# Algolzw/image-restoration-sde

Hardware: AMD Instinct MI355X
Metric: restored images/sec at 256x256, 100-step IR-SDE reverse sampler (higher is better)
Workload: dtype f32; 1 GPU; IR-SDE deraining ConditionalUNet nf=64 depth=4, reverse_sde, batch=16/GPU 256x256, T=100 (BASELINE.json configs[1]); compute_dtype=fp32, global_batch=16

## Files before the change

### image_restoration_sde_amd/_lib.py

```python
import ctypes
import os
import subprocess
import threading

_HERE = os.path.dirname(os.path.abspath(__file__))
LIB_PATH = os.environ.get("IRSDE_LIB_PATH") or os.path.join(_HERE, "libirsde_hip.so")
CSRC = os.path.join(_HERE, "csrc")

MODE = {"sde": 0, "ode": 1, "posterior": 2, "dsde_sde": 3, "dsde_ode": 4}
COEF_STRIDE = 12
FLAG_KEEP_ACTIVATIONS = 1
FLAG_NAIVE_CONV = 2
FLAG_NO_WINOGRAD = 4
FLAG_NO_WINOGRAD_F43 = 8
FLAG_UNCOND_FULLATTN = 16
FLAG_BF16 = 32
FLAG_NAF_INTRO_SKIP = 64
FLAG_BF16_ACT = 128
FLAG_NO_FUSED_LN = 256
FLAG_NAF_LENS = 512
FLAG_FP16 = 1024
FLAG_NO_WINOGRAD_FUSED = 2048
FLAG_NO_FUSED_ATTN = 4096
FLAG_NO_NAF_CHAIN = 8192
FLAG_SPLIT_BF16X2 = 16384
FLAG_SPLIT_F16X2 = 32768
FLAG_NAF_STEREO = 65536
FLAG_NAF_UNCOND = 131072
FLAG_UNET_STEREO = 262144
FLAG_F16_ACT = 524288
FLAG_NO_WINO_POLY = 1048576
FLAG_SCAM_STREAM = 2097152
FLAG_NO_SPLIT3 = 4194304
SAMPLE_GRAPH = 1
SAMPLE_PROFILE = 2

SYMBOLS = [
    "irsde_last_error", "irsde_version", "irsde_create", "irsde_create_nafnet", "irsde_destroy", "irsde_num_weights",
    "irsde_weight_name", "irsde_weight_shape", "irsde_load_weight", "irsde_finalize_weights",
    "irsde_set_schedule", "irsde_unet_forward", "irsde_sample", "irsde_sde_step", "irsde_philox_normal",
    "irsde_get_profile", "irsde_debug_tap", "irsde_work_model", "irsde_debug_conv", "irsde_debug_conv_choice", "irsde_debug_conv_halo_choice", "irsde_debug_conv_features", "irsde_plan_describe", "irsde_bench_conv", "irsde_op_profile", "irsde_debug_split_gemm", "irsde_bench_naf_chain", "irsde_debug_force_subbatches", "irsde_debug_force_chain_groups", "irsde_debug_force_wino_poly", "irsde_debug_force_split3", "irsde_debug_force_split3_attn", "irsde_debug_force_split3_blocks", "irsde_debug_scam", "irsde_debug_scam_full",
    "irsde_debug_scam_stream", "irsde_debug_scam_full_stream", "irsde_debug_force_scam_stream",
    "irsde_debug_naf_gate_sca", "irsde_debug_tlsc", "irsde_debug_ln_film", "irsde_debug_naf_lnconv", "irsde_debug_naf_chain", "irsde_debug_naf_chain_split_order",
    "irsde_debug_full_attention16",
    "irsde_eval_metrics", "irsde_tensor2img", "irsde_upscale_bicubic", "irsde_mask_to", "irsde_imresize",
    "irsde_set_lens_info", "irsde_nafnet_set_local_pool", "irsde_create_latent_unet", "irsde_latent_shapes", "irsde_latent_encode", "irsde_latent_decode", "irsde_latent_hidden",
]


class IrsdeLibraryError(RuntimeError):
    pass


class IrsdeError(RuntimeError):
    pass


class Config(ctypes.Structure):
    _fields_ = [("in_nc", ctypes.c_int32), ("out_nc", ctypes.c_int32), ("nf", ctypes.c_int32),
                ("depth", ctypes.c_int32), ("device", ctypes.c_int32), ("flags", ctypes.c_int32)]


class NafConfig(ctypes.Structure):
    _fields_ = [("img_channel", ctypes.c_int32), ("width", ctypes.c_int32), ("middle_blk_num", ctypes.c_int32),
                ("n_enc", ctypes.c_int32), ("enc_blk_nums", ctypes.c_int32 * 8), ("n_dec", ctypes.c_int32),
                ("dec_blk_nums", ctypes.c_int32 * 8), ("device", ctypes.c_int32), ("flags", ctypes.c_int32)]


class LatentConfig(ctypes.Structure):
    _fields_ = [("in_ch", ctypes.c_int32), ("out_ch", ctypes.c_int32), ("ch", ctypes.c_int32), ("n_mult", ctypes.c_int32),
                ("ch_mult", ctypes.c_int32 * 8), ("embed_dim", ctypes.c_int32), ("device", ctypes.c_int32),
                ("flags", ctypes.c_int32)]


_lib = None
_lock = threading.Lock()


PROBES_LIB_PATH = os.path.join(_HERE, "libirsde_hip_probes.so")


def build_library(force=False, verbose=False, probes=True):
    if force:
        subprocess.run(["make", "-C", CSRC, "clean"], check=True, capture_output=not verbose)
    for extra in ([], ["PROBES=1"]) if probes else ([],):
        r = subprocess.run(["make", "-j8", "-C", CSRC] + extra, capture_output=True, text=True)
        if r.returncode != 0:
            raise IrsdeLibraryError("building libirsde_hip%s.so failed:\n" % ("_probes" if extra else "") + r.stdout + r.stderr)
        if verbose:
            print(r.stdout)
    return LIB_PATH


def _declare(lib):
    c = ctypes
    P = c.c_void_p
    lib.irsde_last_error.restype = c.c_char_p
    lib.irsde_last_error.argtypes = []
    lib.irsde_version.restype = c.c_int
    lib.irsde_create.argtypes = [c.POINTER(Config), c.POINTER(P)]
    lib.irsde_create_nafnet.argtypes = [c.POINTER(NafConfig), c.POINTER(P)]
    lib.irsde_destroy.argtypes = [P]
    lib.irsde_destroy.restype = None
    lib.irsde_num_weights.argtypes = [P]
    lib.irsde_weight_name.argtypes = [P, c.c_int]
    lib.irsde_weight_name.restype = c.c_char_p
    lib.irsde_weight_shape.argtypes = [P, c.c_int, c.POINTER(c.c_int64), c.POINTER(c.c_int)]
    lib.irsde_load_weight.argtypes = [P, c.c_char_p, P, c.POINTER(c.c_int64), c.c_int]
    lib.irsde_finalize_weights.argtypes = [P]
    lib.irsde_set_schedule.argtypes = [P, c.c_int, P]
    lib.irsde_unet_forward.argtypes = [P, P, P, c.POINTER(c.c_int64), c.c_int, c.c_int, c.c_int, c.c_int, P, P]
    lib.irsde_sample.argtypes = [P, c.c_int, P, P, P, c.c_uint64, c.c_uint64, c.c_int, c.c_int, c.c_int,
                                 c.c_int, c.c_int, P, P, c.c_int]
    lib.irsde_sde_step.argtypes = [c.c_int, c.c_int, P, P, P, P, P, c.c_uint64, c.c_uint64, c.c_int, c.c_int,
                                   c.c_int, c.c_int, P]
    lib.irsde_philox_normal.argtypes = [P, c.c_int, c.c_int, c.c_int, c.c_uint64, c.c_uint64, P]
    lib.irsde_get_profile.argtypes = [P, c.POINTER(c.c_double)]
    lib.irsde_debug_tap.argtypes = [P, c.c_char_p, P, c.POINTER(c.c_int64)]
    lib.irsde_work_model.argtypes = [P, c.c_int, c.c_int, c.c_int, c.POINTER(c.c_double)]
    lib.irsde_debug_conv.argtypes = [P, c.c_int, P, c.c_int, c.c_int, c.c_int, c.c_int, c.c_int, P, c.c_int, c.c_int,
                                     c.c_int, c.c_int, c.c_int, P, P, c.c_int, c.c_int, P, P, c.c_int, c.c_int, P]
    lib.irsde_debug_conv_choice.argtypes = [c.c_int] * 13 + [c.c_uint] + [c.c_int] * 4 + [c.POINTER(c.c_int), c.c_char_p, c.c_int]
    lib.irsde_debug_conv_halo_choice.argtypes = [c.c_int] * 13 + [c.c_uint] + [c.c_int] * 5 + [c.c_char_p, c.c_int]
    lib.irsde_debug_conv_features.argtypes = ([P, c.c_int, P, c.c_int] + [c.c_int] * 4 + [P] + [c.c_int] * 7 + [P] * 3 + [P, c.c_int, P, P, P, c.c_int] + [c.c_int] * 6 +
                                              [c.POINTER(c.c_int), P, c.c_char_p, c.c_int, P])
    lib.irsde_plan_describe.argtypes = [P, c.c_int, c.c_int, c.c_int, c.c_char_p, c.c_int]
    lib.irsde_op_profile.argtypes = [P, c.c_char_p, c.c_int]
    lib.irsde_bench_conv.argtypes = [c.c_int] * 11 + [c.POINTER(c.c_double)]
    lib.irsde_bench_naf_chain.argtypes = [c.c_int] * 4 + [c.POINTER(c.c_double)]
    lib.irsde_debug_force_subbatches.argtypes = [c.c_int]
    lib.irsde_debug_force_chain_groups.argtypes = [c.c_int]
    lib.irsde_debug_force_wino_poly.argtypes = [c.c_int]
    lib.irsde_debug_force_split3.argtypes = [c.c_int]
    lib.irsde_debug_force_split3_attn.argtypes = [c.c_int]
    lib.irsde_debug_force_split3_blocks.argtypes = [c.c_int]
    lib.irsde_debug_scam.argtypes = [P, c.c_int, c.c_int, c.c_int, c.c_int] + [P] * 12 + [P, P]
    lib.irsde_debug_scam_full.argtypes = [P, c.c_int, c.c_int, c.c_int, c.c_int] + [P] * 12 + [P, P]
    lib.irsde_debug_scam_stream.argtypes = [P, c.c_int, c.c_int, c.c_int, c.c_int] + [P] * 12 + [c.c_int, P, P]
    lib.irsde_debug_scam_full_stream.argtypes = [P, c.c_int, c.c_int, c.c_int, c.c_int] + [P] * 12 + [c.c_int, P, P]
    lib.irsde_debug_force_scam_stream.argtypes = [c.c_int]
    lib.irsde_debug_naf_gate_sca.argtypes = [P, c.c_int, c.c_int, c.c_int, c.c_int] + [P] * 8
    lib.irsde_debug_tlsc.argtypes = [P] + [c.c_int] * 6 + [P] * 4
    lib.irsde_debug_ln_film.argtypes = [P, c.c_int64, c.c_int, c.c_int64, P, P, P, c.c_int, P, P]
    lib.irsde_debug_naf_lnconv.argtypes = [c.c_int, P, c.c_int64, c.c_int, c.c_int, c.c_int64, P, P, P, c.c_int, P, P, P, c.c_int, P, P, P, P, P]
    lib.irsde_debug_naf_chain.argtypes = [P, P, c.c_int, c.c_int] + [P] * 16 + [P, c.c_int, c.c_int, P, c.c_int, c.c_int, c.c_int, P]
    lib.irsde_debug_naf_chain_split_order.argtypes = [c.c_int, c.c_int, c.POINTER(c.c_int), c.c_int64]
    lib.irsde_debug_full_attention16.argtypes = [P, c.c_int, c.c_int, P, P]
    lib.irsde_debug_split_gemm.argtypes = [P, P, P, c.c_int, c.c_int, c.c_int, c.c_int, c.c_int, P]
    lib.irsde_eval_metrics.argtypes = [P, P, c.c_int, c.c_int, c.c_int, c.c_int, c.c_int, c.POINTER(c.c_double), P]
    lib.irsde_tensor2img.argtypes = [P, P, c.c_int, c.c_int, c.c_int, c.c_int, P]
    lib.irsde_upscale_bicubic.argtypes = [P, P, c.c_int, c.c_int, c.c_int, c.c_int, c.c_int, P]
    lib.irsde_mask_to.argtypes = [P, P, c.c_int, c.c_int, c.c_int, c.c_int, P, c.c_int, c.c_int, c.c_int, c.c_int, P]
    lib.irsde_imresize.argtypes = [P, P] + [c.c_int] * 6 + [P, P, c.c_int, P, P, c.c_int, P]
    lib.irsde_set_lens_info.argtypes =[P, c.POINTER(c.c_float), c.c_int]
    lib.irsde_nafnet_set_local_pool.argtypes = [P, c.c_int, c.c_int, c.c_int, c.c_int]
    lib.irsde_create_latent_unet.argtypes = [c.POINTER(LatentConfig), c.POINTER(P)]
    lib.irsde_latent_shapes.argtypes = [P, c.c_int, c.c_int, c.POINTER(c.c_int64), c.POINTER(c.c_int64), c.POINTER(c.c_int)]
    lib.irsde_latent_encode.argtypes = [P, P, c.c_int, c.c_int, c.c_int, P, c.POINTER(P), P]
    lib.irsde_latent_decode.argtypes = [P, P, c.POINTER(P), c.c_int, c.c_int, c.c_int, P, P]
    lib.irsde_latent_hidden.argtypes = [P, c.c_int, c.c_int, c.c_int, c.c_int, P, P]
    for name in SYMBOLS:
        getattr(lib, name)
    return lib


def lib():
    global _lib
    with _lock:
        if _lib is None:
            if not os.path.exists(LIB_PATH):
                raise IrsdeLibraryError(
                    "libirsde_hip.so not found at %s — build it with `python -c 'import __graft_entry__ as g; "
                    "g.build()'` or `make -C %s`. There is no CPU/PyTorch fallback for this path." % (LIB_PATH, CSRC))
            try:
                _lib = _declare(ctypes.CDLL(LIB_PATH))
            except OSError as ex:
                raise IrsdeLibraryError("failed to load %s: %s" % (LIB_PATH, ex)) from ex
        return _lib


_probes = None


def probes_lib():
    global _probes
    with _lock:
        if _probes is None:
            if not os.path.exists(PROBES_LIB_PATH):
                raise IrsdeLibraryError("libirsde_hip_probes.so not found at %s — build it with `make -C %s PROBES=1`" % (PROBES_LIB_PATH, CSRC))
            try:
                _probes = _declare(ctypes.CDLL(PROBES_LIB_PATH))
            except OSError as ex:
                raise IrsdeLibraryError("failed to load %s: %s" % (PROBES_LIB_PATH, ex)) from ex
        return _probes


def check(rc, L=None):
    if rc != 0:
        msg = (L or lib()).irsde_last_error()
        raise IrsdeError("libirsde_hip error %d: %s" % (rc, msg.decode() if msg else "?"))


def stream_ptr(torch_stream=None):
    import torch
    s = torch_stream if torch_stream is not None else torch.cuda.current_stream()
    return ctypes.c_void_p(s.cuda_stream)
```

### image_restoration_sde_amd/csrc/common.h

```cpp
#pragma once
#include <hip/hip_runtime.h>
#include <cstdint>
#include <cstdio>
#include <cstdlib>
#include <stdexcept>
#include <string>
#include <vector>
#include "split3_layout.h"

namespace irsde {

struct HipError : std::runtime_error {
    using std::runtime_error::runtime_error;
};
struct HipOutOfMemory : HipError {
    using HipError::HipError;
};

inline int tuning_env_int(const char* name, int dflt) {
    static const bool on = [] { const char* t = getenv("IRSDE_TUNING"); return t && atoi(t) == 1; }();
    if (!on) return dflt;
    const char* v = getenv(name);
    return v ? atoi(v) : dflt;
}
// ... 35 lines not shown
    const float* zeros = nullptr;
    const float* ch_scale = nullptr;
    const float* in_scale = nullptr;
    int gate = 0;
    const float* gate_film = nullptr;
    int gate_film_bstride = 0;
    int shuffle = 0;
    int nz = 1;
    long long z_in = 0, z_w = 0, z_out = 0;
    int no_direct_epi = 0;
    int in_bf16 = 0, out_bf16 = 0;
    int in_f16 = 0, out_f16 = 0;
    const float* ln_g = nullptr;
    float ln_eps = 1e-5f;
};

struct WinoParams {
    const float* in0 = nullptr;
    const float* in1 = nullptr;
    int C0 = 0, C1 = 0, Hin = 0, Win = 0, in_shift = 0;
    int B = 0, TH = 0, TW = 0, T = 0;
    int tile = 2;
    float* V = nullptr;
    unsigned short* Vs = nullptr;
    int nplanes = 0;
    int v_f16 = 0;
    float v_scale = 1.f;
    int v_pairs = 0;
    int v_triples = 0;
    const float* M = nullptr;
    int Cout = 0;
    float* out = nullptr;
    int out_stride = 0;
    const float* bias = nullptr;
    const float* film = nullptr;
    int film_bstride = 0;
    int silu = 0;
    const float* res = nullptr;
    int res_stride = 0;
};
void launch_wino_input(const WinoParams& p, hipStream_t s);
struct WinoPolyParams {
    int up = 0;
    const float* in = nullptr;
    int C = 0, Hin = 0, Win = 0;
    int B = 0, TH = 0, TW = 0, T = 0;
    float* V = nullptr;
    unsigned short* Vs = nullptr;
    int thread_writer = 0;
    const float* M = nullptr;
    int Cout = 0, Ho = 0, Wo = 0;
    float* out = nullptr;
    int out_stride = 0;
    const float* bias = nullptr;
};
void launch_wino_poly_input(const WinoPolyParams& p, hipStream_t s);
void launch_wino_poly_output(const WinoPolyParams& p, hipStream_t s);
void wino_poly_transform_weights(const float* w_packed, int Cout, int Cin, float* U, int up);
struct SplitGemmArgs {
    const unsigned short* a = nullptr;
    const unsigned short* b = nullptr;
    float* out = nullptr;
    long long plA = 0, plB = 0, pA = 0, pB = 0, pO = 0;
    int M = 0, N = 0, K = 0, lda = 0, ldc = 0;
    float out_scale = 1.f;
    int n_inner = 1;
    int nblk_n = 0;
};
void gemm_split_global_init();
void launch_gemm_split_pairs(const SplitGemmArgs& a, int ncomp, hipStream_t s, int abl = 0, bool f16 = false);
void launch_split_pairs(const float* in, unsigned short* out, size_t rows, int K, hipStream_t s, bool f16 = false,
                        float scale = 1.0f);
struct Split3Launch {
    enum Abl { FULL = 0, NO_LOADS = 1, NO_MFMA = 3, NO_STORES = 4 };
    enum Tri { RULE, ON, OFF };
    Abl abl = FULL;
    Tri walk = RULE;
    Tri drain = RULE;
};
void launch_gemm_split_triples(const SplitGemmArgs& a, int ncomp, hipStream_t s, const Split3Launch& o = {});
void set_force_split3_blocks(int n);
bool gemm_split_triples_fits(long long M, long long N, long long K, long long ldc);
void launch_split_triples(const float* in, unsigned short* out, int ncomp, size_t rows, int K, hipStream_t s);
void launch_split_planes(const float* in, unsigned short* out, size_t n, size_t plane, int nplanes, hipStream_t s, bool f16 = false,
                         float scale = 1.0f);
void launch_wino_output(const WinoParams& p, hipStream_t s);
void wino_transform_weights(const float* w_packed, int Cout, int Cin, float* U, int tile);
bool wino_fused_eligible(const ConvParams& p);
void wino_fused_pack_weights(const float* U, int Cout, int Cin, float* Uf);
void launch_wino_fused(const ConvParams& p, const float* Uf, hipStream_t s, unsigned long long* dbg = nullptr, int dflags = 0);
int wino_fused_num_blocks(const ConvParams& p);
bool wino_fused64_eligible(const ConvParams& p);
void wino_fused64_pack_weights(const float* U, int Cout, int Cin, float* Uf);
void launch_wino_fused64(const ConvParams& p, const float* Uf, hipStream_t s, int variant = 0);
void wino_fused64_set_debug(unsigned long long* buf);
constexpr float kWinoFused64PairVScale = 0.0625f;
void launch_wino_fused64_split_weights(const float* Uf, unsigned short* out, size_t nfloats, float scale, hipStream_t s);
int wino_fused64_num_blocks(const ConvParams& p);
bool wino_fused64_xcd_nb(const ConvParams& p);
void wino_fused_global_init();
int device_cu_count();
bool wino_fused64t_eligible(const ConvParams& p);
long long wino_fused64t_num_items(const ConvParams& p);
void launch_wino_fused64t(const ConvParams& p, const float* Uf, hipStream_t s, int variant = 0);
void wino_fused64t_set_debug(unsigned long long* buf);
void wino_fused_t_global_init();
void naf_chain_global_init();
void naf_chain_set_debug(unsigned long long* buf);
bool naf_chain_shape_ok(int H, int W, int c);
size_t naf_chain_weight_halves(int nblocks);
size_t naf_chain_vec_floats(int nblocks);
void launch_naf_chain(const float* x, float* out, const unsigned short* w, const float* vecs, int nblocks, int B, const float* film, int film_bstride,
                      int film_off, const float* cam, int cam_bstride, int cam_off, hipStream_t s, int variant = 0);
std::vector<int> naf_chain_split_order(int nblocks, int G);
void naf_chain_build_split_weights(const unsigned short* w1, unsigned short* dst, int nblocks, int G, hipStream_t s);
size_t naf_chain_split_scratch_bytes(int B);
int naf_chain_split_groups(int B, int G);
void launch_naf_chain_split(const float* x, float* out, const unsigned short* wG, const float* vecs, int nblocks, int B, const float* film, int film_bstride,
                            int film_off, const float* cam, int cam_bstride, int cam_off, int G, void* scratch, hipStream_t s);
const unsigned* naf_chain_split_error_flag(const void* scratch, int B);
void naf_chain_split_reset(void* scratch, int B);
void naf_chain_set_sabotage(int on);
void attention_global_init();

double conv_flops(const ConvParams& p);
struct ConvTune {
    enum Tile { TILE_AUTO, TILE_128, TILE_256x128, TILE_256, TILE_128_ONE_PER_CU };
    enum Halo { HALO_AUTO, HALO_OFF, HALO_FORCE_512, HALO_FORCE_256 };
    enum ZLoop { ZLOOP_AUTO, ZLOOP_OFF, ZLOOP_ALL, ZLOOP_PAIRS, ZLOOP_FORCE_1X1 };
    enum Order { ORDER_AUTO, ORDER_N_FAST, ORDER_N_SLOW };
    bool rules_off = false;
    Tile tile = TILE_AUTO;
    bool no_buffer_desc = false;
    bool no_direct_epi = false;
    Halo halo = HALO_AUTO;
    ZLoop zloop = ZLOOP_AUTO;
    Order halo_order = ORDER_AUTO;
};
struct ConvKnobs {
    int small_bn = 2, small_bn_f32 = 0;
    int pair_tile256 = 1, pair_inscale256 = 0;
    int no_bufa = 0;
    int zloop = -1, zloop_1x1 = -1;
    int zloop_maxnk = 32, zloop_minblk = 1024, zloop_deep = 1, zloop_ragged64 = 2048;
};
const ConvKnobs& conv_knobs_from_env();
struct HaloChoice {
    int pixels = 0;
    int BN = 0;
    int op = 0, act = 0;
    int tiles_x = 0, tiles_y = 0, nblk_n = 0;
    int n_slow = 0;
    unsigned grid = 0;
    int lds = 0;
    int instance = -1;
};
constexpr int kHaloInstances = 9;
struct ConvChoice {
    enum Family { PAIR, NARROW3, ZLOOP_BATCH, ZLOOP_1X1, HALO, IGEMM };
    enum Operand { OP_F32, OP_F32_BUF, OP_BF16, OP_F16 };
    enum Storage { ACT_F32, ACT_BF16, ACT_F16 };
    Family family = IGEMM;
    int BM = 0, BN = 0;
    Operand op = OP_F32;
    Storage act = ACT_F32;
    bool inscale = false;
// ... 167 lines not shown
```

### image_restoration_sde_amd/csrc/engine.h

```cpp
#pragma once
#include <algorithm>
#include <cmath>
#include <cstring>
#include <functional>
#include <map>
#include <memory>
#include <mutex>
#include <string>
#include <vector>

#include "../../include/irsde_hip.h"
#include "common.h"

namespace irsde {

constexpr int kWinoFusedMaxCin = 256, kWinoFusedMaxCout = 256;
inline long long wino_fused_min_tiles() { return tuning_env_int("IRSDE_WINO_FUSED_MINT", 4096); }
inline bool wino_fused64_enabled() { return tuning_env_int("IRSDE_WINO_FUSED64", 1) != 0; }
inline bool wino_fused64_pair_enabled() { return tuning_env_int("IRSDE_WINO_FUSED64_PAIR", 1) != 0; }
inline int wino_fused64_max_cin() { return tuning_env_int("IRSDE_WINO_FUSED64_MAXCIN", 512); }
inline int wino_fused64_max_cout() { return tuning_env_int("IRSDE_WINO_FUSED64_MAXCOUT", 512); }
inline long long wino_fused64_min_tiles() { return tuning_env_int("IRSDE_WINO_FUSED64_MINT", 1024); }
inline int wino_fused64t_mode() { return tuning_env_int("IRSDE_WINO_FUSED64T", 1); }
inline bool naf_lnconv_enabled() { return tuning_env_int("IRSDE_NAF_LNCONV", 1) != 0; }
inline int naf_chain_split_mode() { return tuning_env_int("IRSDE_NAF_CHAIN_SPLIT", 0); }

int wino_poly_mode();
void set_force_wino_poly(int mode);
constexpr int kWinoPolyUpMinCin = 512;
inline bool wino_poly_wants_weights(int mode, bool up, int Cin) { return mode >= 2 || (mode == 1 && (!up || Cin >= kWinoPolyUpMinCin)); }

int split3_mode();
void set_force_split3(int mode);
constexpr int kSplit3WinoMinCin = 512;
inline int split3_wino_min_cin() { return tuning_env_int("IRSDE_SPLIT3_MINCIN", kSplit3WinoMinCin); }
inline bool split3_wino_wants_weights(int mode, int Cin, int Cout) { return mode >= 2 || Cin > 512 || (Cin >= split3_wino_min_cin() && Cout >= 512); }
inline long long split3_fused_min_tiles() { return tuning_env_int("IRSDE_SPLIT3_FUSED_MINT", 4096); }
constexpr int kSplit3NotExactF32 = IRSDE_FLAG_NO_WINOGRAD | IRSDE_FLAG_NAIVE_CONV | IRSDE_FLAG_BF16 | IRSDE_FLAG_BF16_ACT | IRSDE_FLAG_FP16 | IRSDE_FLAG_F16_ACT |
                                   IRSDE_FLAG_SPLIT_BF16X2 | IRSDE_FLAG_SPLIT_F16X2 | IRSDE_FLAG_NO_SPLIT3;
inline bool split3_wants_weights(int flags) { return !(flags & kSplit3NotExactF32) && split3_mode() > 0; }
int split3_attn_mode();
void set_force_split3_attn(int mode);

inline int wino_min_c(int tile) {
    return tuning_env_int(tile == 4 ? "IRSDE_WINO4_MINC" : "IRSDE_WINO2_MINC", tile == 4 ? 64 : 256);
}

struct DeviceScope {
    int prev = -1;
    explicit DeviceScope(int dev) {
        if (hipGetDevice(&prev) != hipSuccess) prev = -1;
        if (prev != dev) IRSDE_HIP_CHECK(hipSetDevice(dev));
        else prev = -1;
    }
    ~DeviceScope() {
        if (prev >= 0) (void)hipSetDevice(prev);
    }
    DeviceScope(const DeviceScope&) = delete;
    DeviceScope& operator=(const DeviceScope&) = delete;
};

struct HostTensor {
    std::vector<int64_t> shape;
    std::vector<float> data;
    bool loaded = false;
};

struct ConvW {
    float* w = nullptr;
    float* bias = nullptr;
    int Cout = 0, Cin = 0, KH = 1, KW = 1;
    float* wino_u2 = nullptr;
    float* wino_u4 = nullptr;
    float* wino_uf = nullptr;
    float* wino_uf64 = nullptr;
    unsigned short* wino_uf64p = nullptr;
    float wino_uf64p_scale = 1.f;
    unsigned short* wino_up = nullptr;
    float wino_up_scale = 1.f;
    unsigned short* wino_u4t = nullptr;
    unsigned short* wino_polyt = nullptr;
    float* wino_poly = nullptr;
};
struct ResW {
    ConvW b1, b2, res;
    bool has_res = false;
    float* mlp_w = nullptr;
    float* mlp_b = nullptr;
    int film_off = 0;
    int Cout = 0;
};
struct ScamW {
    int c = 0;
    float *gl = nullptr, *gr = nullptr;
    ConvW l, r;
    float *beta = nullptr, *gamma = nullptr;
};
struct AttnW {
    float* g1 = nullptr;
    ConvW qkv, out;
    float* g2 = nullptr;
    int C = 0;
};

struct NafBlockW {
    int c = 0;
    float *g1 = nullptr, *g2 = nullptr;
    ConvW conv1, conv3, conv4, conv5;
    float *dw_w = nullptr, *dw_b = nullptr;
    float *sca_w = nullptr, *sca_b = nullptr;
    float *beta = nullptr, *gamma = nullptr;
    float *mlp_w = nullptr, *mlp_b = nullptr;
    int film_off = 0;
    float *cam_w = nullptr, *cam_b = nullptr;
    int cam_off = 0;
    ScamW fusion;
};

struct NafChainW {
    unsigned short* w = nullptr;
    float* vecs = nullptr;
    int nblocks = 0, film_off = 0, cam_off = 0;
    unsigned short* wsplit[5] = {nullptr, nullptr, nullptr, nullptr, nullptr};
};

// ... 226 lines not shown
    ScamW mid_scam;
    std::vector<ResW> up_res;
    std::vector<AttnW> up_attn;
    std::vector<ConvW> up_conv;
    ResW final_res;
    std::vector<ResW*> all_res;
    int film_row = 0;

    int arch = 0;
    int naf_ic = 0;
    std::vector<int> naf_enc_nums, naf_dec_nums;
    int naf_mid_num = 0;
    std::vector<std::vector<NafBlockW>> naf_enc, naf_dec;
    std::vector<NafBlockW> naf_mid;
    std::vector<ConvW> naf_downs, naf_ups;
    ConvW naf_intro, naf_ending;
    std::vector<NafBlockW*> naf_all;
    std::vector<NafChainW> naf_chain_enc, naf_chain_dec;
    NafChainW naf_chain_mid;
    float *cm_w1 = nullptr, *cm_b1 = nullptr, *cm_w3 = nullptr, *cm_b3 = nullptr;
    int cam_row = 0;
    float* cam_cur = nullptr;
    int cam_rows = 0;
    int cam_set = 0;

    int tlsc_base_h = 0, tlsc_base_w = 0, tlsc_train_h = 0, tlsc_train_w = 0;

    int lat_in = 0, lat_out = 0, lat_ch = 0, lat_embed = 0;
    std::vector<int> lat_mult;
    ConvW lat_init, lat_latent, lat_post, lat_final;
    std::vector<ResW> lat_enc_res, lat_dec_res;
    AttnW lat_enc_attn, lat_dec_attn;
    std::vector<ConvW> lat_down, lat_up;
    std::vector<std::unique_ptr<LatentPlan>> lat_plans;

    int T = 0;
    float* coef_table = nullptr;
    float* film_table = nullptr;
    float* film_cur = nullptr;
    int film_cur_rows = 0;
    StepState* step = nullptr;
    SampleCtl* ctl = nullptr;

    float* zeros = nullptr;
    hipStream_t stream = nullptr;
    hipEvent_t ev_in = nullptr, ev_out = nullptr;
    static constexpr int kMaxSub = 4;
    hipStream_t sub_stream[kMaxSub - 1] = {nullptr, nullptr, nullptr};
    hipEvent_t ev_fork = nullptr, ev_join[kMaxSub - 1] = {nullptr, nullptr, nullptr};
    std::vector<std::unique_ptr<Plan>> plans;
    uint64_t use_counter = 0;
    double profile[12] = {0};
    std::vector<double> op_ms;
    std::vector<std::string> op_desc;
    int op_steps = 0;
    int plan_parts = 1;
    int op_split = 1;
    std::vector<hipEvent_t> ev_pool;
    std::mutex mu;

    float* dmalloc(size_t n) {
        float* p = nullptr;
        IRSDE_HIP_CHECK(hipMalloc(&p, std::max<size_t>(n, 16) * sizeof(float)));
        dev_allocs.push_back(p);
        return p;
    }
    std::map<const float*, unsigned short*> bf16_copies;
    const unsigned short* bf16_copy(const float* w, size_t n) {
        auto it = bf16_copies.find(w);
        if (it != bf16_copies.end()) return it->second;
        unsigned short* d = nullptr;
        IRSDE_HIP_CHECK(hipMalloc(&d, n * sizeof(unsigned short)));
        if (cfg.flags & IRSDE_FLAG_FP16) launch_f32_to_f16(w, d, n, stream);
        else launch_f32_to_bf16(w, d, n, stream);
        IRSDE_HIP_CHECK(hipStreamSynchronize(stream));
        bf16_copies[w] = d;
        return d;
    }
    struct PairCopy { unsigned short* p; float inv_scale; };
    std::map<const float*, PairCopy> pair_copies;
    PairCopy pair_copy(const float* w, size_t n) {
        return make_pair_copy(pair_copies, w, n, [&](unsigned short* d, bool f16, float sc) { launch_split_planes(w, d, n, n, 2, stream, f16, sc); });
    }
    std::map<const float*, unsigned short*> triple_copies;
    const unsigned short* triple_copy(const float* w, size_t rows, int K) {
        const size_t n = rows * (size_t)K;
        auto it = triple_copies.find(w);
        if (it != triple_copies.end()) return it->second;
        unsigned short* d = nullptr;
        IRSDE_HIP_CHECK(hipMalloc(&d, 3 * n * sizeof(unsigned short)));
        dev_allocs.push_back(reinterpret_cast<float*>(d));
        launch_split_frag3(w, d, rows, K, stream);
        IRSDE_HIP_CHECK(hipStreamSynchronize(stream));
        triple_copies[w] = d;
        return d;
    }
    std::map<const float*, PairCopy> pair_copies_il;
    PairCopy pair_copy_il(const float* w, size_t rows, int K) {
        return make_pair_copy(pair_copies_il, w, rows * (size_t)K, [&](unsigned short* d, bool f16, float sc) { launch_split_pairs(w, d, rows, K, stream, f16, sc); });
    }
    template <class Split>
    PairCopy make_pair_copy(std::map<const float*, PairCopy>& cache, const float* w, size_t n, Split split) {
        auto it = cache.find(w);
        if (it != cache.end()) return it->second;
        const bool f16 = (cfg.flags & IRSDE_FLAG_SPLIT_F16X2) != 0;
        float sc = 1.f;
        if (f16) {
            std::vector<float> h(n);
            IRSDE_HIP_CHECK(hipMemcpy(h.data(), w, n * sizeof(float), hipMemcpyDeviceToHost));
            sc = pow2_scale_into_512(h.data(), n);
        }
        unsigned short* d = nullptr;
        IRSDE_HIP_CHECK(hipMalloc(&d, 2 * n * sizeof(unsigned short)));
        dev_allocs.push_back(reinterpret_cast<float*>(d));
        split(d, f16, sc);
        IRSDE_HIP_CHECK(hipStreamSynchronize(stream));
        const PairCopy pc{d, 1.0f / sc};
        cache[w] = pc;
        return pc;
    }
    float* upload(const std::vector<float>& v) {
        float* p = dmalloc(v.size());
        IRSDE_HIP_CHECK(hipMemcpy(p, v.data(), v.size() * sizeof(float), hipMemcpyHostToDevice));
        return p;
    }
};

namespace irsde {

inline bool naf_lens(const irsde_engine* e) { return (e->cfg.flags & IRSDE_FLAG_NAF_LENS) != 0; }
inline bool naf_stereo(const irsde_engine* e) { return e->arch == 1 && (e->cfg.flags & IRSDE_FLAG_NAF_STEREO) != 0; }
inline bool unet_stereo(const irsde_engine* e) { return e->arch == 0 && (e->cfg.flags & IRSDE_FLAG_UNET_STEREO) != 0; }
inline bool stereo_engine(const irsde_engine* e) { return naf_stereo(e) || unet_stereo(e); }
inline bool uncond_engine(const irsde_engine* e) {
    return (e->arch == 0 && (e->cfg.flags & IRSDE_FLAG_UNCOND_FULLATTN) != 0) || (e->arch == 1 && (e->cfg.flags & IRSDE_FLAG_NAF_UNCOND) != 0);
}
inline int rup32(int c) { return (c + 31) & ~31; }
inline bool tlsc_window(const irsde_engine* e, int level, int* K0, int* K1) {
    if (e->tlsc_train_h <= 0) return false;
    const int P = 1 << e->cfg.depth;
    const int Hp = (e->tlsc_train_h + P - 1) / P * P, Wp = (e->tlsc_train_w + P - 1) / P * P;
    *K0 = (int)((long long)(Hp >> level) * e->tlsc_base_h / e->tlsc_train_h);
    *K1 = (int)((long long)(Wp >> level) * e->tlsc_base_w / e->tlsc_train_w);
    return true;
}
inline StepState* step_of(const irsde_engine* e, const Plan* pl) { return pl->own_step ? pl->own_step : e->step; }
inline float* film_of(const irsde_engine* e, const Plan* pl) { return pl->own_film ? pl->own_film : e->film_cur; }

void build_inventory(irsde_engine* e);
void build_inventory_naf(irsde_engine* e);
void build_inventory_latent(irsde_engine* e);
void finalize(irsde_engine* e);
void compute_film_rows(irsde_engine* e, const float* tvals, int rows, float* dst, hipStream_t s);
void ensure_film_cur(irsde_engine* e, int rows);
void pack_conv_rows(const float* w_oihw, const float* bias, int O, int I, int KH, int KW, const std::vector<int>& perm, std::vector<float>& pw,
                    std::vector<float>& pb);
std::vector<int> naf_gate_perm(int c);
std::vector<int> naf_shuffle_perm(int Cout);
std::vector<float> pack_dwconv_taps(const float* w, int c2);
void pack_naf_chain_host(const std::vector<NafChainHostW>& blocks, std::vector<unsigned short>& w, std::vector<float>& vecs);

Plan* get_plan(irsde_engine* e, int B, int H, int W, bool per_sample_film, int slot = 0, int b0 = 0);
int naf_subbatches(const irsde_engine* e, int B, int H, int W);
void set_force_chain_groups(int g);
void set_force_scam_stream(int block_w);
int forced_chain_groups();
int forced_scam_stream();
void set_force_subbatches(int n);
LatentPlan* get_latent_plan(irsde_engine* e, int B, int H, int W, bool decode);

int guard(const std::function<void()>& f);

}
```

### image_restoration_sde_amd/csrc/engine_debug.hip

```cpp
#include "engine.h"
#include "../../include/irsde_hip_debug.h"

using namespace irsde;

namespace irsde {
namespace {

struct Scratch {
    hipStream_t s;
    std::vector<void*> bufs;
    explicit Scratch(hipStream_t s_) : s(s_) {}
    ~Scratch() {
        (void)hipStreamSynchronize(s);
        for (void* p : bufs) (void)hipFree(p);
    }
    Scratch(const Scratch&) = delete;
    Scratch& operator=(const Scratch&) = delete;
    template <class T> T* alloc(size_t n) {
        void* p = nullptr;
        IRSDE_HIP_CHECK(hipMalloc(&p, n * sizeof(T)));
        bufs.push_back(p);
        return static_cast<T*>(p);
    }
    float* upload(const float* host, size_t n) {
// ... 4 lines not shown
    float* upload(const std::vector<float>& v) { return upload(v.data(), v.size()); }
};
struct OwnedStream {
    hipStream_t s = nullptr;
    explicit OwnedStream(unsigned flags) { IRSDE_HIP_CHECK(hipStreamCreateWithFlags(&s, flags)); }
    ~OwnedStream() { (void)hipStreamDestroy(s); }
    OwnedStream(const OwnedStream&) = delete;
    OwnedStream& operator=(const OwnedStream&) = delete;
};
struct EventPair {
    hipEvent_t e0 = nullptr, e1 = nullptr;
    EventPair() {
        IRSDE_HIP_CHECK(hipEventCreate(&e0));
        IRSDE_HIP_CHECK(hipEventCreate(&e1));
    }
    ~EventPair() {
        if (e0) (void)hipEventDestroy(e0);
        if (e1) (void)hipEventDestroy(e1);
    }
    EventPair(const EventPair&) = delete;
    EventPair& operator=(const EventPair&) = delete;
};
template <class Run>
double time_launches(hipStream_t s, int iters, Run&& run) {
    EventPair ev;
    IRSDE_HIP_CHECK(hipEventRecord(ev.e0, s));
    for (int i = 0; i < iters; ++i) run();
    IRSDE_HIP_CHECK(hipEventRecord(ev.e1, s));
    IRSDE_HIP_CHECK(hipStreamSynchronize(s));
    float ms = 0.f;
    IRSDE_HIP_CHECK(hipEventElapsedTime(&ms, ev.e0, ev.e1));
    return ms / iters;
}


ConvTune conv_tune_from_code(int code) {
    ConvTune t;
    t.rules_off = code != 0;
    switch (code) {
        case 3: t.tile = ConvTune::TILE_256x128; break;
        case 50: t.tile = ConvTune::TILE_256; break;
        case 5: t.tile = ConvTune::TILE_128_ONE_PER_CU; break;
        case 6: t.no_buffer_desc = true; break;
        case 7: t.no_direct_epi = true; break;
        case 60: t.tile = ConvTune::TILE_256; t.halo = ConvTune::HALO_OFF; break;
        case 61: t.tile = ConvTune::TILE_128; t.halo = ConvTune::HALO_OFF; break;
        case 64: t.halo = ConvTune::HALO_FORCE_512; break;
        case 65: t.halo = ConvTune::HALO_FORCE_256; break;
        case 68: t.halo = ConvTune::HALO_FORCE_512; t.halo_order = ConvTune::ORDER_N_SLOW; break;
        case 69: t.halo = ConvTune::HALO_FORCE_256; t.halo_order = ConvTune::ORDER_N_SLOW; break;
        case 70: t.zloop = ConvTune::ZLOOP_OFF; break;
        case 71: t.zloop = ConvTune::ZLOOP_ALL; break;
        case 72: t.zloop = ConvTune::ZLOOP_PAIRS; break;
        case 73: t.zloop = ConvTune::ZLOOP_FORCE_1X1; break;
        default: break;
    }
    return t;
}

Split3Launch split3_launch_twin(int twin, int abl = 0) {
    Split3Launch o;
    o.abl = static_cast<Split3Launch::Abl>(abl);
    o.walk = twin == 0 ? Split3Launch::RULE : twin == 1 ? Split3Launch::OFF : Split3Launch::ON;
    o.drain = twin == 0 ? Split3Launch::RULE : twin == 1 ? Split3Launch::OFF : Split3Launch::ON;
    return o;
}

enum class Operand { F32, BF16, F16 };

enum class ConvPath {
    Direct,
    Valu,
    WinoF2,
    WinoF4,
    Poly,
    PolyTriples,
    F4Triples,
    F4Pairs,
    DirectPair,
    Fused32,
    Fused64,
    Fused64Pair,
    Fused64T,
};
struct DebugConvRow {
    int code;
    ConvPath path;
    Operand op;
    bool act_bf16;
    int tune;
    int variant;
    bool up;
    bool thread_writer;
};
constexpr DebugConvRow direct(int code, Operand op, bool act_bf16, int tune) { return {code, ConvPath::Direct, op, act_bf16, tune, 0, false, false}; }
constexpr DebugConvRow on_path(int code, ConvPath path, Operand op = Operand::F32) { return {code, path, op, false, 0, 0, false, false}; }
constexpr DebugConvRow wino(int code, ConvPath path, int tune) { return {code, path, Operand::F32, false, tune, 0, false, false}; }
constexpr DebugConvRow poly(int code, ConvPath path, bool up, bool thread_writer = false) { return {code, path, Operand::F32, false, 0, 0, up, thread_writer}; }
constexpr DebugConvRow fused(int code, ConvPath path, int variant) { return {code, path, Operand::F32, false, 0, variant, false, false}; }
constexpr DebugConvRow kDebugConv[] = {
    direct(0, Operand::F32, false, 0),
    on_path(1, ConvPath::Valu),
    wino(2, ConvPath::WinoF2, 0), wino(12, ConvPath::WinoF2, 71), wino(22, ConvPath::WinoF2, 72),
    wino(3, ConvPath::WinoF4, 0), wino(13, ConvPath::WinoF4, 71), wino(23, ConvPath::WinoF4, 72),
    poly(24, ConvPath::Poly, false), poly(25, ConvPath::Poly, true),
    poly(26, ConvPath::PolyTriples, false), poly(27, ConvPath::PolyTriples, true), poly(28, ConvPath::PolyTriples, true, true),
    on_path(48, ConvPath::F4Triples),
    on_path(44, ConvPath::F4Pairs, Operand::F16), on_path(45, ConvPath::F4Pairs, Operand::BF16),
    on_path(46, ConvPath::DirectPair, Operand::F16), on_path(47, ConvPath::DirectPair, Operand::BF16),
    on_path(33, ConvPath::Fused32),
    fused(34, ConvPath::Fused64, 0), fused(36, ConvPath::Fused64, 64), fused(55, ConvPath::Fused64, 20),
    fused(35, ConvPath::Fused64Pair, 4), fused(37, ConvPath::Fused64Pair, 4 + 64), fused(56, ConvPath::Fused64Pair, 24),
    fused(62, ConvPath::Fused64T, 0), fused(63, ConvPath::Fused64T, 64),
    direct(4, Operand::BF16, false, 0), direct(160, Operand::BF16, false, 60), direct(161, Operand::BF16, false, 61), direct(162, Operand::BF16, false, 64),
    direct(163, Operand::BF16, false, 65),
    direct(5, Operand::F16, false, 0), direct(165, Operand::F16, false, 61), direct(166, Operand::F16, false, 64), direct(167, Operand::F16, false, 65),
    direct(204, Operand::BF16, true, 0), direct(260, Operand::BF16, true, 60), direct(261, Operand::BF16, true, 61), direct(262, Operand::BF16, true, 64),
    direct(263, Operand::BF16, true, 65),
    direct(100, Operand::F32, false, 0), direct(103, Operand::F32, false, 3), direct(105, Operand::F32, false, 5), direct(106, Operand::F32, false, 6),
    direct(107, Operand::F32, false, 7), direct(150, Operand::F32, false, 50), direct(170, Operand::F32, false, 70), direct(171, Operand::F32, false, 71),
    direct(172, Operand::F32, false, 72), direct(173, Operand::F32, false, 73),
};

enum class BenchKind {
    Conv,
    Fused32,
    Fused32Stamps,
    Wino3,
    Wino3Gemm,
    Fused64,
    Fused64Stamps,
    Fused64T,
    Fused64TStamps,
    PairGemm,
    TripleGemm,
};
struct BenchRow {
    int lo, hi;
    BenchKind kind;
    int arg;
    Operand op;
    bool pair;
    bool act_bf16;
};
constexpr BenchRow bench(int lo, int hi, BenchKind kind, int arg, Operand op = Operand::F32, bool pair = false, bool act_bf16 = false) {
    return {lo, hi, kind, arg, op, pair, act_bf16};
}
constexpr BenchRow kBenchConv[] = {
    bench(0, 0, BenchKind::Conv, 0), bench(3, 3, BenchKind::Conv, 3), bench(5, 7, BenchKind::Conv, 5), bench(50, 50, BenchKind::Conv, 50),
    bench(70, 73, BenchKind::Conv, 70),
    bench(60, 61, BenchKind::Conv, 60, Operand::BF16),
    bench(62, 62, BenchKind::Conv, 0, Operand::BF16),
    bench(63, 63, BenchKind::Conv, 0, Operand::BF16, false, true),
    bench(64, 65, BenchKind::Conv, 64, Operand::BF16),
    bench(66, 67, BenchKind::Conv, 64, Operand::BF16, false, true),
    bench(480, 480, BenchKind::Conv, 0, Operand::F16, true), bench(481, 481, BenchKind::Conv, 0, Operand::BF16, true),
    bench(482, 482, BenchKind::Conv, 61, Operand::F16, true),
    bench(80, 80, BenchKind::Fused32, 0),
    bench(83, 82 + 255, BenchKind::Fused32, 1),
    bench(82, 82, BenchKind::Fused32Stamps, 0),
    bench(81, 81, BenchKind::Wino3, 0), bench(421, 421, BenchKind::Wino3Gemm, 0),
    bench(430, 432, BenchKind::Fused64, 20),
    bench(434, 434, BenchKind::Fused64, 24, Operand::F16),
    bench(435, 435, BenchKind::Fused64Stamps, 25), bench(2004, 2004, BenchKind::Fused64Stamps, 25),
    bench(2001, 2002, BenchKind::Fused64Stamps, 28),
    bench(460, 462, BenchKind::Fused64T, 0),
    bench(467, 469, BenchKind::Fused64T, 6),
    bench(465, 465, BenchKind::Fused64TStamps, 5),
    bench(4650, 4653, BenchKind::Fused64TStamps, 12),
    bench(472, 476, BenchKind::PairGemm, 0),
    bench(490, 504, BenchKind::TripleGemm, 0),
};

template <class Row, size_t N, class Lo, class Hi>
constexpr bool codes_disjoint(const Row (&rows)[N], Lo lo, Hi hi) {
    for (size_t i = 0; i < N; ++i)
        for (size_t j = 0; j < N; ++j)
            if (i != j && lo(rows[i]) <= hi(rows[j]) && lo(rows[j]) <= hi(rows[i])) return false;
    return true;
}
constexpr int row_code(const DebugConvRow& r) { return r.code; }
constexpr int row_lo(const BenchRow& r) { return r.lo; }
constexpr int row_hi(const BenchRow& r) { return r.hi; }
static_assert(codes_disjoint(kDebugConv, row_code, row_code), "irsde_debug_conv: a selector code has two rows");
static_assert(codes_disjoint(kBenchConv, row_lo, row_hi), "irsde_bench_conv: a variant has two rows");

const DebugConvRow& debug_conv_lookup(int code) {
    for (const DebugConvRow& r : kDebugConv)
        if (r.code == code) return r;
    throw HipError("debug_conv: unknown selector code " + std::to_string(code));
}
struct BenchSel {
    const BenchRow& row;
    int arg;
};
BenchSel bench_conv_lookup(int code) {
    for (const BenchRow& r : kBenchConv)
        if (code >= r.lo && code <= r.hi) return {r, r.arg + (code - r.lo)};
    throw HipError("bench_conv: unknown variant " + std::to_string(code));
}

SplitGemmArgs split_gemm_args(const unsigned short* a, const unsigned short* b, float* C, int M, int N, int K, size_t pA, size_t pB) {
    SplitGemmArgs g;
    g.a = a; g.b = b; g.out = C;
    g.pA = (long long)pA; g.pB = (long long)pB; g.pO = (long long)M * N;
    g.M = M; g.N = N; g.K = K; g.lda = K; g.ldc = N;
    return g;
}
SplitGemmArgs split_triples(Scratch& mem, const float* A, const float* Bm, float* C, int M, int N, int K, int ncomp, hipStream_t s) {
    const size_t ea = split3_comp_elems((size_t)M, (size_t)K), eb = split3_comp_elems((size_t)N, (size_t)K);
    unsigned short *ta = mem.alloc<unsigned short>(ea * ncomp), *tb = mem.alloc<unsigned short>(eb * ncomp);
    launch_split_triples(A, ta, ncomp, (size_t)M, K, s);
    launch_split_triples(Bm, tb, ncomp, (size_t)N, K, s);
    return split_gemm_args(ta, tb, C, M, N, K, ea, eb);
}
SplitGemmArgs split_pairs(Scratch& mem, const float* A, const float* Bm, float* C, int M, int N, int K, int ncomp, hipStream_t s, bool f16 = false, float sa = 1.f,
                          float sb = 1.f) {
    unsigned short *pa = mem.alloc<unsigned short>((size_t)2 * ncomp * M * K), *pb = mem.alloc<unsigned short>((size_t)2 * ncomp * N * K);
    launch_split_pairs(A, pa, (size_t)ncomp * M, K, s, f16, sa);
    launch_split_pairs(Bm, pb, (size_t)ncomp * N, K, s, f16, sb);
    SplitGemmArgs g = split_gemm_args(pa, pb, C, M, N, K, (size_t)M * K, (size_t)N * K);
    g.out_scale = 1.0f / (sa * sb);
    return g;
}

void write_choice_line(const ConvChoice& c, char* out, int out_len) {
    snprintf(out, (size_t)out_len, "name=%s family=%d tile=%dx%d op=%d act=%d inscale=%d zbatch=%d zrows=%d grid=%ux%ux%u threads=%d lds=%d row=%d of %d",
             c.name().c_str(), (int)c.family, c.BM, c.BN, (int)c.op, (int)c.act, (int)c.inscale, c.zbatch, c.zrows, c.gx, c.gy, c.gz, c.threads, c.lds, c.row,
             conv_instance_count());
}

void write_halo_line(const HaloChoice& h, char* out, int out_len) {
    snprintf(out, (size_t)out_len, "kernel=halo%d bn=%d op=%d act=%d tiles=%dx%d nblk_n=%d nslow=%d grid=%u lds=%d instance=%d of %d", h.pixels, h.BN, h.op, h.act,
             h.tiles_x, h.tiles_y, h.nblk_n, h.n_slow, h.grid, h.lds, h.instance, kHaloInstances);
}

ConvParams choice_hook_params(int B, int Hin, int Win, int C0, int C1, int Cout, int K, int stride, int pad, int in_shift, int operand, int storage, int pair,
                              unsigned features, int splits, int nz) {
    static const float dummy[4] = {};
    float* const some = const_cast<float*>(dummy);
    auto bit = [&](int i) { return (features >> i & 1u) ? some : nullptr; };
    ConvParams p;
    p.in0 = some; p.C0 = C0; p.pix0 = C0; p.in1 = C1 ? some : nullptr; p.C1 = C1; p.pix1 = C1;
    p.Hin = Hin; p.Win = Win; p.in_shift = in_shift;
    p.w = some; p.Cout = Cout; p.KH = K; p.KW = K; p.stride = stride; p.pad_y = pad; p.pad_x = pad;
    p.B = B;
    p.Ho = ((Hin << in_shift) + 2 * pad - K) / stride + 1;
    p.Wo = ((Win << in_shift) + 2 * pad - K) / stride + 1;
    p.out = some; p.out_stride = Cout; p.res_stride = Cout; p.zeros = some;
    p.bias = bit(0); p.film = bit(1); p.silu = bit(2) != nullptr; p.res = bit(3); p.in_scale = bit(4); p.ch_scale = bit(5);
    p.gate = bit(6) != nullptr; p.shuffle = bit(7) != nullptr; p.ln_g = bit(8);
    if (pair) p.w_pair = reinterpret_cast<const unsigned short*>(some);
    else if (operand) p.w_bf = reinterpret_cast<const unsigned short*>(some);
    p.f16 = operand == 2;
// ... 306 lines not shown
        const int Cin = C0 + C1;
        std::vector<float> pk((size_t)Cout * KH * KW * Cin);
        for (int o = 0; o < Cout; ++o)
            for (int i = 0; i < Cin; ++i)
                for (int ky = 0; ky < KH; ++ky)
                    for (int kx = 0; kx < KW; ++kx)
                        pk[(((size_t)o * KH + ky) * KW + kx) * Cin + i] = w_oihw[(((size_t)o * Cin + i) * KH + ky) * KW + kx];
        Scratch mem(s);
        float* dw = mem.upload(pk);
        float* db = bias ? mem.upload(bias, Cout) : nullptr;
        ConvParams p;
        p.in0 = in0; p.C0 = C0; p.pix0 = C0; p.in1 = in1; p.C1 = C1; p.pix1 = C1;
        p.Hin = Hin; p.Win = Win; p.in_shift = in_shift;
        p.w = dw; p.Cout = Cout; p.KH = KH; p.KW = KW; p.stride = stride; p.pad_y = pad; p.pad_x = pad;
        p.B = B;
        p.Ho = ((Hin << in_shift) + 2 * pad - KH) / stride + 1;
        p.Wo = ((Win << in_shift) + 2 * pad - KW) / stride + 1;
        p.out = out; p.out_stride = Cout; p.bias = db; p.film = film; p.film_bstride = film_bstride; p.silu = silu;
        p.res = res; p.res_stride = Cout;
        float* dz = mem.alloc<float>(256);
        IRSDE_HIP_CHECK(hipMemset(dz, 0, 1024));
        p.zeros = dz;
        if (splits > 1 && r.path != ConvPath::Valu && r.path != ConvPath::WinoF2 && r.path != ConvPath::WinoF4) {
            p.splits = splits;
            p.partial = mem.alloc<float>((size_t)splits * B * p.Ho * p.Wo * Cout);
        }
        auto wino_weights = [&](int tile) {
            std::vector<float> U((size_t)(tile + 2) * (tile + 2) * Cout * Cin);
            wino_transform_weights(pk.data(), Cout, Cin, U.data(), tile);
            return U;
        };
        auto wino_tiles = [&](int tile) { return (long long)B * (p.Ho / tile) * (p.Wo / tile); };
        auto alloc_M = [&](int ncomp, long long T) { return mem.alloc<float>((size_t)ncomp * T * Cout); };
        auto poly_plan = [&](const char* refusal, float*& dU) {
            if (!(r.up ? wino_poly_up_shape(p) : wino_poly_down_shape(p)) || !wino_poly_eligible(p) || splits > 1) throw HipError(refusal);
            std::vector<float> U((size_t)100 * Cout * Cin);
            wino_poly_transform_weights(pk.data(), Cout, Cin, U.data(), r.up);
            dU = mem.upload(U);
            return make_wino_poly(p, dU, nullptr, nullptr);
        };
        switch (r.path) {
        case ConvPath::PolyTriples: {
            float* dU = nullptr;
            WinoPolyPlan wp = poly_plan("debug_conv: selectors 26 / 27 / 28 run what 24 / 25 run (single source, channels a multiple of 32, bias only)", dU);
            if (!gemm_split_triples_fits(wp.T, Cout, wp.K, Cout)) throw HipError("debug_conv: shape not eligible for the three-piece GEMM");
            unsigned short* dUt = mem.alloc<unsigned short>((size_t)wp.ncomp * split3_comp_elems((size_t)Cout, (size_t)wp.K));
            unsigned short* dVt = mem.alloc<unsigned short>((size_t)wp.ncomp * split3_comp_elems((size_t)wp.T, (size_t)wp.K));
            float* dM = alloc_M(wp.ncomp, wp.T);
            launch_split_triples(dU, dUt, wp.ncomp, (size_t)Cout, wp.K, s);
            wp = make_wino_poly(p, dU, nullptr, dM);
            const SplitGemmArgs sg = make_wino_poly_triples(wp, Cout, dUt, dVt, dM);
            wp.in.thread_writer = r.thread_writer;
            launch_wino_poly_input(wp.in, s);
            launch_gemm_split_triples(sg, wp.ncomp, s);
            launch_wino_poly_output(wp.out, s);
            break;
        }
        case ConvPath::Poly: {
            float* dU = nullptr;
            WinoPolyPlan wp = poly_plan(r.up ? "debug_conv: selector 25 runs a 3x3 stride-1 pad-1 convolution with in_shift = 1 (single source, channels a multiple of 32, bias only)"
                                             : "debug_conv: selector 24 runs a 4x4 stride-2 pad-1 convolution (single source, channels a multiple of 32, bias only)", dU);
            float* dV = mem.alloc<float>((size_t)wp.ncomp * wp.T * wp.K);
            wp = make_wino_poly(p, dU, dV, alloc_M(wp.ncomp, wp.T));
            launch_wino_poly_input(wp.in, s);
            launch_conv(wp.gemm, s);
            launch_wino_poly_output(wp.out, s);
            break;
        }
        case ConvPath::F4Triples: {
            if (!wino_shape_ok(p, 4) || Cin % 32) throw HipError("debug_conv: shape not eligible for the three-piece GEMM");
            const std::vector<float> U = wino_weights(4);
            const long long T = wino_tiles(4);
            if (!gemm_split_triples_fits(T, Cout, Cin, Cout)) throw HipError("debug_conv: shape not eligible for the three-piece GEMM");
            float* dU = mem.upload(U);
            unsigned short* dUt = mem.alloc<unsigned short>((size_t)36 * split3_comp_elems((size_t)Cout, (size_t)Cin));
            unsigned short* dVt = mem.alloc<unsigned short>((size_t)36 * split3_comp_elems((size_t)T, (size_t)Cin));
            launch_split_triples(dU, dUt, 36, (size_t)Cout, Cin, s);
            const WinoSplitPlan sp = make_wino_triples(p, dUt, dVt, alloc_M(36, T));
            launch_wino_input(sp.in, s);
            launch_gemm_split_triples(sp.gemm, 36, s);
            launch_wino_output(sp.out, s);
            break;
        }
        case ConvPath::F4Pairs: {
            const bool f16 = r.op == Operand::F16;
            if (!wino_shape_ok(p, 4) || Cin % 32) throw HipError("debug_conv: shape not eligible for the pair GEMM");
            std::vector<float> U = wino_weights(4);
            const float us = f16 ? pow2_scale_into_512(U.data(), U.size()) : 1.f;
            const long long T = wino_tiles(4);
            float* dU = mem.upload(U);
            unsigned short* dUp = mem.alloc<unsigned short>(2 * U.size());
            unsigned short* dVp = mem.alloc<unsigned short>((size_t)36 * T * Cin * 2);
            launch_split_pairs(dU, dUp, (size_t)36 * Cout, Cin, s, f16, us);
            const WinoSplitPlan sp = make_wino_pairs(p, dUp, dVp, alloc_M(36, T), f16, us);
            launch_wino_input(sp.in, s);
            launch_gemm_split_pairs(sp.gemm, 36, s, 0, f16);
            launch_wino_output(sp.out, s);
            break;
        }
        case ConvPath::Fused64Pair: {
            if (!wino_fused64_eligible(p)) throw HipError("debug_conv: shape not eligible for the fused Winograd kernel");
            std::vector<float> U = wino_weights(4), Uf(U.size());
            wino_fused64_pack_weights(U.data(), Cout, Cin, Uf.data());
            const float usc = pow2_scale_into_512(U.data(), U.size());
            float* dUf = mem.upload(Uf);
            unsigned short* dUp = mem.alloc<unsigned short>(2 * Uf.size());
            launch_wino_fused64_split_weights(dUf, dUp, Uf.size(), usc, s);
            p.pair_scale = 1.0f / (kWinoFused64PairVScale * usc);
            launch_wino_fused64(p, reinterpret_cast<const float*>(dUp), s, r.variant);
            break;
        }
        case ConvPath::Fused32:
        case ConvPath::Fused64:
        case ConvPath::Fused64T: {
            const bool f32k = r.path == ConvPath::Fused32;
            if (f32k ? !wino_fused_eligible(p) : !wino_fused64_eligible(p)) throw HipError("debug_conv: shape not eligible for the fused Winograd kernel");
            const std::vector<float> U = wino_weights(4);
            std::vector<float> Uf(U.size());
            if (f32k) wino_fused_pack_weights(U.data(), Cout, Cin, Uf.data());
            else wino_fused64_pack_weights(U.data(), Cout, Cin, Uf.data());
            float* dUf = mem.upload(Uf);
            if (r.path == ConvPath::Fused64T) {
                if (!wino_fused64t_eligible(p)) throw HipError("debug_conv: shape not eligible for the two-tile-group fused Winograd kernel");
                launch_wino_fused64t(p, dUf, s, r.variant);
            } else if (f32k) {
                launch_wino_fused(p, dUf, s);
            } else {
                launch_wino_fused64(p, dUf, s, r.variant);
            }
            break;
        }
        case ConvPath::WinoF2:
        case ConvPath::WinoF4: {
            const int tile = r.path == ConvPath::WinoF2 ? 2 : 4, ncomp = (tile + 2) * (tile + 2);
            if (!wino_shape_ok(p, tile)) throw HipError("debug_conv: shape not eligible for Winograd");
            const std::vector<float> U = wino_weights(tile);
            const long long T = wino_tiles(tile);
            float* dU = mem.upload(U);
            float* dV = mem.alloc<float>((size_t)ncomp * T * Cin);
            const WinoPlan wp = make_wino(p, dU, dV, alloc_M(ncomp, T), tile);
            launch_wino_input(wp.in, s);
            launch_conv(wp.gemm, s, conv_tune_from_code(r.tune));
            launch_wino_output(wp.out, s);
            break;
        }
        case ConvPath::DirectPair: {
            const bool f16 = r.op == Operand::F16;
            const float sc = f16 ? pow2_scale_into_512(pk.data(), pk.size()) : 1.f;
            unsigned short* dwp = mem.alloc<unsigned short>(2 * pk.size());
            launch_split_pairs(dw, dwp, (size_t)Cout, KH * KW * (C0 + C1), s, f16, sc);
            p.w_pair = dwp; p.pair_scale = 1.0f / sc; p.f16 = f16 ? 1 : 0;
            launch_conv(p, s);
            break;
        }
        case ConvPath::Valu:
            launch_conv_naive(p, s);
            break;
        case ConvPath::Direct: {
            unsigned short* ao = nullptr;
            if (r.op != Operand::F32) {
                unsigned short* d16 = mem.alloc<unsigned short>(pk.size());
                if (r.op == Operand::F16) launch_f32_to_f16(dw, d16, pk.size(), s);
                else launch_f32_to_bf16(dw, d16, pk.size(), s);
                p.w_bf = d16;
                p.f16 = r.op == Operand::F16 ? 1 : 0;
            }
// ... 112 lines not shown
            wsc = f16 ? pow2_scale_into_512(pk.data(), pk.size()) : 1.f;
            w16 = mem.alloc<unsigned short>(2 * pk.size());
            p.w_pair = w16; p.pair_scale = 1.0f / wsc;
        } else if (operand) {
            w16 = mem.alloc<unsigned short>(pk.size());
            p.w_bf = w16;
        }
        p.f16 = f16 ? 1 : 0;
        if (storage) {
            a0 = mem.alloc<unsigned short>(npix_in * C0);
            p.in0 = reinterpret_cast<const float*>(a0);
            if (in1) { a1 = mem.alloc<unsigned short>(npix_in * C1); p.in1 = reinterpret_cast<const float*>(a1); }
            if (res) { ar = mem.alloc<unsigned short>(nout); p.res = reinterpret_cast<const float*>(ar); }
            ao = mem.alloc<unsigned short>(nout);
            p.out = reinterpret_cast<float*>(ao);
            p.in_bf16 = p.out_bf16 = storage == 1;
            p.in_f16 = p.out_f16 = storage == 2;
        }
        ConvKnobs k;
        static_assert(sizeof(ConvKnobs) == 11 * sizeof(int), "the hook's knob array is ConvKnobs, field by field");
        if (knobs) memcpy(&k, knobs, sizeof k);
        conv_validate(p);
        auto narrow = [&](const float* src, unsigned short* dst, size_t n) {
            if (storage == 2) launch_f32_to_f16(src, dst, n, s);
            else launch_f32_to_bf16(src, dst, n, s);
        };
        if (pair) launch_split_pairs(dw, w16, (size_t)Cout * nz, K * K * Cin, s, f16, wsc);
        else if (operand == 2) launch_f32_to_f16(dw, w16, pk.size(), s);
        else if (operand == 1) launch_f32_to_bf16(dw, w16, pk.size(), s);
        if (storage) {
            narrow(in0, a0, npix_in * C0);
            if (in1) narrow(in1, a1, npix_in * C1);
            if (res) narrow(res, ar, nout);
            IRSDE_HIP_CHECK(hipMemsetAsync(ao, 0xFF, nout * 2, s));
        }
        ConvChoice c;
        launch_conv(p, s, conv_tune_from_code(tune), knobs ? &k : nullptr, &c);
        if (storage == 2) launch_f16_to_f32(ao, out, nout, s);
        else if (storage == 1) launch_bf16_to_f32(ao, out, nout, s);
        IRSDE_HIP_CHECK(hipStreamSynchronize(s));
        write_choice_line(c, choice, choice_len);
        if (c.family == ConvChoice::HALO) {
            const size_t n = strlen(choice);
            if (n + 2 < (size_t)choice_len) {
                choice[n] = ' ';
                write_halo_line(c.halo, choice + n + 1, choice_len - (int)n - 1);
            }
        }
    });
}

int irsde_debug_split_gemm(const float* A, const float* Bm, float* C, int M, int N, int K, int ncomp, int nplanes, void* stream) {
    return guard([&] {
        const int twin3 = nplanes == 43 ? 0 : nplanes == 45 ? 1 : nplanes == 47 ? 2 : -1;
        if (twin3 < 0 && nplanes != 42 && nplanes != 44) throw HipError("debug_split_gemm: nplanes must be 42, 43, 44, 45 or 47");
        hipStream_t s = reinterpret_cast<hipStream_t>(stream);
        conv_global_init();
        Scratch mem(s);
        if (twin3 >= 0) {
            if (!gemm_split_triples_fits(M, N, K, N)) throw HipError("debug_split_gemm: shape not eligible for the three-piece GEMM");
            launch_gemm_split_triples(split_triples(mem, A, Bm, C, M, N, K, ncomp, s), ncomp, s, split3_launch_twin(twin3));
        } else {
            const bool f16 = nplanes == 44;
            launch_gemm_split_pairs(split_pairs(mem, A, Bm, C, M, N, K, ncomp, s, f16, f16 ? 1.0f / 16.0f : 1.f, f16 ? 64.0f : 1.f), ncomp, s, 0, f16);
        }
        IRSDE_HIP_CHECK(hipStreamSynchronize(s));
    });
}

int irsde_debug_force_chain_groups(int g) {
    set_force_chain_groups(g == 1 || g == 2 || g == 4 ? g : 0);
    return IRSDE_OK;
}

int irsde_debug_force_split3(int mode) {
    set_force_split3(mode >= 0 && mode <= 2 ? mode : -1);
    return IRSDE_OK;
}

int irsde_debug_force_split3_attn(int mode) {
    set_force_split3_attn(mode >= 0 && mode <= 2 ? mode : -1);
    return IRSDE_OK;
}
int irsde_debug_force_split3_blocks(int n) {
    if (n >= 0 && n < 8) return guard([&] { throw HipError("debug_force_split3_blocks: n must be at least 8 (one block per XCD), or negative for the default"); });
    set_force_split3_blocks(n);
    return IRSDE_OK;
}

int irsde_debug_force_wino_poly(int mode) {
    set_force_wino_poly(mode >= 0 && mode <= 2 ? mode : -1);
    return IRSDE_OK;
}

int irsde_debug_force_subbatches(int n) {
    set_force_subbatches(n < 0 ? 0 : n);
    return IRSDE_OK;
}

int irsde_bench_naf_chain(int variant, int nblocks, int B, int iters, double* ms_out) {
    return guard([&] {
        if (!ms_out || nblocks < 1 || nblocks > 64 || B < 1 || iters < 1) throw HipError("bench_naf_chain: bad argument");
        const int G = variant == 22 ? 2 : (variant == 24 || variant == 25 || variant == 26) ? 4 : 1;
#ifdef IRSDE_PROBES
        if (variant != 0 && variant != 1 && variant != 11 && G == 1) throw HipError("bench_naf_chain: bad variant");
#else
        if (variant != 0 && variant != 1 && G == 1) throw HipError("bench_naf_chain: variant 11 is a measurement twin (make PROBES=1)");
#endif
        conv_global_init();
        OwnedStream stream(hipStreamDefault);
        hipStream_t s = stream.s;
        Scratch mem(s);
        const size_t nx = (size_t)B * 64 * 512, nw = naf_chain_weight_halves(nblocks), nv = naf_chain_vec_floats(nblocks);
        float *dx = mem.alloc<float>(nx), *dout = mem.alloc<float>(nx), *dvec = mem.alloc<float>(nv), *dfilm = mem.alloc<float>((size_t)nblocks * 2048);
        unsigned short* dw = mem.alloc<unsigned short>(nw);
        const size_t chunk = (size_t)64 << 20;
        float* dwf = mem.alloc<float>(chunk);
        launch_fill_random(dx, nx, 1, 1.0f, s);
        launch_fill_random(dvec, nv, 2, 0.1f, s);
        launch_fill_random(dfilm, (size_t)nblocks * 2048, 3, 0.1f, s);
        for (size_t o = 0; o < nw; o += chunk) {
            const size_t n = std::min(chunk, nw - o);
            launch_fill_random(dwf, n, 4 + (unsigned)(o / chunk), 0.04f, s);
            launch_f32_to_f16(dwf, dw + o, n, s);
        }
        unsigned short* dwg = nullptr;
        void* dscratch = nullptr;
        if (G > 1) {
            IRSDE_HIP_CHECK(hipStreamSynchronize(s));
            dwg = mem.alloc<unsigned short>(nw);
            naf_chain_build_split_weights(dw, dwg, nblocks, G, s);
            dscratch = mem.alloc<char>(naf_chain_split_scratch_bytes(B));
            IRSDE_HIP_CHECK(hipMemset(dscratch, 0, naf_chain_split_scratch_bytes(B)));
        }
        auto run = [&]() {
            if (G > 1) launch_naf_chain_split(dx, dout, dwg, dvec, nblocks, B, dfilm, 0, 0, nullptr, 0, 0, G, dscratch, s);
            else launch_naf_chain(dx, dout, dw, dvec, nblocks, B, dfilm, 0, 0, nullptr, 0, 0, s, variant == 11 ? 1 : variant);
        };
        if (variant == 26) {
#ifdef IRSDE_PROBES
            naf_chain_set_sabotage(1);
#else
            throw HipError("bench_naf_chain: variant 26 is a PROBES-build test");
#endif
        }
        struct SabotageOff { ~SabotageOff() { naf_chain_set_sabotage(0); } } sabotage_off;
        run();
        if (variant == 25) {
#ifdef IRSDE_PROBES
            const int ng = naf_chain_split_groups(B, 4);
            unsigned long long* dd = mem.alloc<unsigned long long>((size_t)ng * 8 * 16);
            IRSDE_HIP_CHECK(hipMemsetAsync(dd, 0, (size_t)ng * 8 * 16 * 8, s));
            naf_chain_set_debug(dd);
            run();
            IRSDE_HIP_CHECK(hipStreamSynchronize(s));
            naf_chain_set_debug(nullptr);
            std::vector<unsigned long long> hd((size_t)ng * 8 * 16);
            IRSDE_HIP_CHECK(hipMemcpy(hd.data(), dd, hd.size() * 8, hipMemcpyDeviceToHost));
            double acc[16] = {0};
            double nwv = 0;
            for (size_t w = 0; w < (size_t)ng * 8; ++w) {
                if (!hd[w * 16 + 15]) continue;
                for (int k = 0; k < 16; ++k) acc[k] += (double)hd[w * 16 + k];
                nwv += 1;
            }
            static const char* names[12] = {"norm1 (incl. residual-stream fetch)", "conv1 GEMM passes", "depthwise 3x3 + gate + pool", "gated fetch behind barrier (pool)", "sca.1 GEMM", "conv3 GEMM + residual", "norm2 (incl. residual-stream fetch)", "conv4 GEMM + gate", "conv5 GEMM + residual", "scale-vector / gated fetch (sca, conv4)", "group barriers (6 per block)", "publishing (gated slice, residual slice)"};
            printf("naf_chain stamps, 4 groups per image: %d blocks, B=%d; shader cycles per wave and block (mean over %.0f waves)\n", nblocks, B, nwv);
            for (int k = 0; k < 12; ++k) printf("  %-42s %9.0f\n", names[k], acc[k] / nwv / nblocks);
            printf("  %-42s %9.0f\n", "whole kernel / blocks", acc[15] / nwv / nblocks);
            fflush(stdout);
#else
            throw HipError("bench_naf_chain: variant 25 is a measurement twin (make PROBES=1)");
#endif
        }
        if (variant == 11) {
            unsigned long long* dd = mem.alloc<unsigned long long>((size_t)B * 8 * 16);
            IRSDE_HIP_CHECK(hipMemsetAsync(dd, 0, (size_t)B * 8 * 16 * 8, s));
            naf_chain_set_debug(dd);
            launch_naf_chain(dx, dout, dw, dvec, nblocks, B, dfilm, 0, 0, nullptr, 0, 0, s, 11);
            IRSDE_HIP_CHECK(hipStreamSynchronize(s));
            naf_chain_set_debug(nullptr);
            std::vector<unsigned long long> hd((size_t)B * 8 * 16);
            IRSDE_HIP_CHECK(hipMemcpy(hd.data(), dd, hd.size() * 8, hipMemcpyDeviceToHost));
            double acc[16] = {0};
            for (size_t i = 0; i < hd.size(); ++i) acc[i % 16] += (double)hd[i];
            const double nwv = (double)B * 8, nb = nblocks;
            static const char* names[10] = {"norm1", "conv1 GEMM passes", "depthwise 3x3 + gate + pool", "barrier (pool)", "sca.1 GEMM", "conv3 GEMM + residual", "norm2", "conv4 GEMM + gate", "conv5 GEMM + residual", "barriers (sca, conv4)"};
            printf("naf_chain stamps: %d blocks, B=%d; shader cycles per wave and block (mean over %d waves); MFMA floor per wave: conv1 / conv4 512 x 16, conv3 / conv5 256 x 16, sca 64 x 16\n", nblocks, B, B * 8);
            for (int k = 0; k < 10; ++k) printf("  %-30s %9.0f\n", names[k], acc[k] / nwv / nb);
            printf("  %-30s %9.0f\n", "whole kernel / blocks", acc[15] / nwv / nb);
            fflush(stdout);
        }
        *ms_out = time_launches(s, iters, run);
        if (G > 1) {
            unsigned flag = 0;
            IRSDE_HIP_CHECK(hipMemcpy(&flag, naf_chain_split_error_flag(dscratch, B), 4, hipMemcpyDeviceToHost));
            if (flag) throw HipError("bench_naf_chain: the split kernel's groups were not co-resident (spin timeout)");
        }
    });
}

int irsde_bench_conv(int variant, int B, int H, int W, int Cin, int Cout, int K, int stride, int up, int epi, int iters,
                     double* ms_out) {
    return guard([&] {
        if (!ms_out || iters < 1) throw HipError("bad argument");
        const BenchSel sel = bench_conv_lookup(variant);
        const BenchRow& r = sel.row;
        const BenchKind kind = r.kind;
        const int arg = sel.arg;
        conv_global_init();
        OwnedStream stream(hipStreamNonBlocking);
        hipStream_t s = stream.s;
        Scratch mem(s);
        ConvParams p;
        p.B = B; p.Hin = H; p.Win = W; p.in_shift = up; p.C0 = Cin; p.pix0 = Cin;
        p.Cout = Cout; p.KH = K; p.KW = K; p.stride = stride; p.pad_y = p.pad_x = (K == 4 ? 1 : K / 2);
        p.Ho = ((H << up) + 2 * p.pad_y - K) / stride + 1;
        p.Wo = ((W << up) + 2 * p.pad_x - K) / stride + 1;
        const size_t nin = (size_t)B * H * W * Cin, nw = (size_t)Cout * K * K * Cin, nout = (size_t)B * p.Ho * p.Wo * Cout;
        float *din = mem.alloc<float>(nin), *dw = mem.alloc<float>(nw), *dout = mem.alloc<float>(nout), *dres = mem.alloc<float>(nout);
        float* dfilm = mem.alloc<float>((size_t)2 * Cout + 256);
        float* dz = dfilm + 2 * Cout;
        IRSDE_HIP_CHECK(hipMemset(dz, 0, 1024));
        p.zeros = dz;
        launch_fill_random(din, nin, 1, 1.0f, s);
        launch_fill_random(dw, nw, 2, 1.0f / sqrtf((float)(K * K * Cin)), s);
        launch_fill_random(dres, nout, 3, 1.0f, s);
        launch_fill_random(dfilm, (size_t)2 * Cout, 4, 0.3f, s);
        p.in0 = din; p.w = dw; p.out = dout; p.out_stride = Cout;
        if (kind == BenchKind::Conv && r.op == Operand::BF16 && !r.pair) {
            unsigned short* dbf = mem.alloc<unsigned short>(nw);
            launch_f32_to_bf16(dw, dbf, nw, s);
            p.w_bf = dbf;
        }
        if (epi == 1) { p.film = dfilm; p.silu = 1; }
        if (epi == 2) { p.silu = 1; p.res = dres; p.res_stride = Cout; }
        if (r.act_bf16) {
            unsigned short* dabf = mem.alloc<unsigned short>(nin);
            launch_f32_to_bf16(din, dabf, nin, s);
            launch_f32_to_bf16(dout, reinterpret_cast<unsigned short*>(dres), nout / 2, s);
            p.in0 = reinterpret_cast<const float*>(dabf);
            p.in_bf16 = 1; p.out_bf16 = 1;
        }
        if (r.pair) {
            const bool f16 = r.op == Operand::F16;
            unsigned short* dwp = mem.alloc<unsigned short>(2 * nw);
            launch_split_pairs(dw, dwp, (size_t)Cout, K * K * Cin, s, f16, 64.0f);
            p.w_pair = dwp; p.pair_scale = 1.0f / 64.0f; p.f16 = f16 ? 1 : 0;
        }
        if (kind == BenchKind::TripleGemm || kind == BenchKind::PairGemm) {
            if (K != 3 || stride != 1 || !wino_shape_ok(p, 4)) throw HipError("bench_conv: Winograd variants need an eligible 3x3 stride-1 layer");
            const long long T = (long long)B * (p.Ho / 4) * (p.Wo / 4);
            const bool triples = kind == BenchKind::TripleGemm;
            if (triples && !gemm_split_triples_fits(T, Cout, Cin, Cout)) throw HipError("bench_conv: shape not eligible for the three-piece GEMM");
            float *vf = mem.alloc<float>((size_t)36 * T * Cin), *uf = mem.alloc<float>((size_t)36 * Cout * Cin), *mo = mem.alloc<float>((size_t)36 * T * Cout);
            launch_fill_random(vf, (size_t)36 * T * Cin, 7, 1.0f, s);
            launch_fill_random(uf, (size_t)36 * Cout * Cin, 8, 0.05f, s);
            const SplitGemmArgs g = triples ? split_triples(mem, vf, uf, mo, (int)T, Cout, Cin, 36, s) : split_pairs(mem, vf, uf, mo, (int)T, Cout, Cin, 36, s);
            const Split3Launch twin = split3_launch_twin(arg / 5, arg % 5);
            auto gemms = [&] {
                if (triples) launch_gemm_split_triples(g, 36, s, twin);
                else launch_gemm_split_pairs(g, 36, s, arg);
            };
            for (int i = 0; i < 2; ++i) gemms();
            *ms_out = time_launches(s, iters, gemms);
            return;
        }
        float* dU = nullptr;
        WinoPlan wp{};
        if (kind == BenchKind::Fused32Stamps) {
            dU = mem.alloc<float>((size_t)36 * nw / 9);
            launch_fill_random(dU, (size_t)36 * nw / 9, 5, 1.0f / sqrtf((float)(9 * Cin)), s);
            const int nb = wino_fused_num_blocks(p);
            unsigned long long* dd = mem.alloc<unsigned long long>((size_t)nb * 128);
            launch_wino_fused(p, dU, s);
            IRSDE_HIP_CHECK(hipMemsetAsync(dd, 0, (size_t)nb * 128 * 8, s));
            launch_wino_fused(p, dU, s, dd);
            IRSDE_HIP_CHECK(hipStreamSynchronize(s));
            std::vector<unsigned long long> hd((size_t)nb * 128);
            IRSDE_HIP_CHECK(hipMemcpy(hd.data(), dd, hd.size() * 8, hipMemcpyDeviceToHost));
            double ph[2][4] = {{0, 0, 0, 0}, {0, 0, 0, 0}};
            unsigned long long rt_min = ~0ull, rt_max = 0;
            for (int bi = 0; bi < nb; ++bi)
                for (int w = 0; w < 8; ++w) {
                    const unsigned long long* t = &hd[((size_t)bi * 8 + w) * 16];
                    for (int k = 0; k < 4; ++k) ph[w >= 4][k] += (double)(t[k + 1] - t[k]) / ((double)nb * 4);
                    rt_min = std::min(rt_min, t[7]);
                    rt_max = std::max(rt_max, t[7]);
                }
            printf("wino_fused timeline B=%d %dx%d Cin=%d Cout=%d: %d blocks, block starts span %.1f us\n", B, p.Ho, p.Wo, Cin, Cout, nb,
                   (double)(rt_max - rt_min) / 100.0);
            printf("  MFMA waves     (shader cycles): start->V[0] ready %.0f | K loop %.0f | acc->LDS+barrier %.0f | epilogue %.0f\n", ph[0][0],
                   ph[0][1], ph[0][2], ph[0][3]);
            printf("  producer waves (shader cycles): start->chunk 0 done %.0f | K loop rest %.0f | wait MFMA+acc %.0f | epilogue %.0f\n",
                   ph[1][0], ph[1][1], ph[1][2], ph[1][3]);
            fflush(stdout);
            *ms_out = 0.0;
            return;
        }
        if (kind != BenchKind::Conv) {
            const bool three_launch = kind == BenchKind::Wino3 || kind == BenchKind::Wino3Gemm;
            if (K != 3 || stride != 1) throw HipError("bench_conv: Winograd variants need a 3x3 stride-1 layer");
            dU = mem.alloc<float>((size_t)36 * nw / 9);
            launch_fill_random(dU, (size_t)36 * nw / 9, 5, 1.0f / sqrtf((float)(9 * Cin)), s);
            if (!three_launch && !wino_fused_eligible(p)) throw HipError("bench_conv: shape not eligible for the fused Winograd kernel");
            if (kind != BenchKind::Fused32 && kind != BenchKind::Wino3 && !wino_fused64_eligible(p))
                throw HipError("bench_conv: shape not eligible for the 64-cout fused Winograd kernel");
            if (kind == BenchKind::Fused64 && r.op == Operand::F16) {
                float* dUp = mem.alloc<float>((size_t)36 * nw / 9);
                launch_wino_fused64_split_weights(dU, reinterpret_cast<unsigned short*>(dUp), (size_t)36 * nw / 9, 256.0f, s);
                dU = dUp;
                p.pair_scale = 1.0f / (kWinoFused64PairVScale * 256.0f);
            }
            if (three_launch) {
                if (!wino_shape_ok(p, 4)) throw HipError("bench_conv: shape not eligible for Winograd F(4x4,3x3)");
                const long long T = (long long)B * (p.Ho / 4) * (p.Wo / 4);
                float* dV = mem.alloc<float>((size_t)36 * T * Cin);
                float* dM = mem.alloc<float>((size_t)36 * T * Cout);
                wp = make_wino(p, dU, dV, dM, 4);
                if (kind == BenchKind::Wino3Gemm) launch_wino_input(wp.in, s);
            }
        }
        if (kind == BenchKind::Fused64TStamps) {
            if (!wino_fused64t_eligible(p)) throw HipError("bench_conv: shape not eligible for the two-tile-group fused Winograd kernel");
            const int nbp = 256;
            unsigned long long* dd = mem.alloc<unsigned long long>((size_t)nbp * 64);
            launch_wino_fused64t(p, dU, s, 0);
            IRSDE_HIP_CHECK(hipMemsetAsync(dd, 0, (size_t)nbp * 64 * 8, s));
            wino_fused64t_set_debug(dd);
            launch_wino_fused64t(p, dU, s, arg);
            IRSDE_HIP_CHECK(hipStreamSynchronize(s));
// ... 79 lines not shown
```

### image_restoration_sde_amd/csrc/engine_plan.hip

```cpp
#include "engine.h"
#include <atomic>

using namespace irsde;

namespace irsde {

struct Builder {
    irsde_engine* e;
    Plan* pl;
    bool reuse;
    bool naive;
    int film_bstride;
    int b0 = 0;
    const float* film_base() const { return film_of(e, pl) + (size_t)b0 * film_bstride; }
    const float* cam_base() const { return e->cam_cur + (size_t)b0 * e->cam_row; }
    const float* fused_ln_g = nullptr;

    bool act_bf16() const { return (e->cfg.flags & IRSDE_FLAG_BF16_ACT) != 0; }
    bool act_f16() const { return (e->cfg.flags & IRSDE_FLAG_F16_ACT) != 0; }
    Tensor talloc(int B, int H, int W, int C, int force_f32 = 0) {
        Tensor t;
        t.B = B; t.H = H; t.W = W; t.C = C;
        t.bf16 = act_bf16() && !force_f32;
        t.f16 = act_f16() && !force_f32;
        t.p = pl->alloc(t.half() ? (t.numel() + 1) / 2 : t.numel(), reuse);
        return t;
    }
    void tfree(const Tensor& t) {
        if (reuse) pl->release(t.p);
    }
    void tap(const std::string& name, const Tensor& t) { pl->taps[name] = t; }

    void push_op(Op op) {
        pl->conv_flops += op.flops;
        pl->conv_exec_flops += op.exec_flops;
        pl->conv_bytes += op.bytes;
        pl->net_ops.push_back(std::move(op));
    }

    void push_conv(ConvParams p) {
        const int M = p.B * p.Ho * p.Wo;
        const int bn = conv_base_bn(p.Cout);
        const int blocks = ((M + 127) / 128) * ((p.Cout + bn - 1) / bn);
        const int nk = p.KH * p.KW * ((p.C0 + p.C1) / 32);
        int splits = 1;
        if (!naive && blocks < 256 && nk >= 16 && !p.gate && !p.shuffle) {
            splits = std::min(std::min(nk / 8, (512 + blocks - 1) / blocks), 16);
            if (splits < 2) splits = 1;
        }
        if (splits > 1) {
            p.splits = splits;
            p.partial = pl->alloc((size_t)splits * M * p.Cout, true);
        }
        p.zeros = e->zeros;
        if (!naive && (e->cfg.flags & IRSDE_FLAG_BF16)) {
            p.w_bf = e->bf16_copy(p.w, (size_t)p.Cout * p.KH * p.KW * (p.C0 + p.C1));
            p.f16 = (e->cfg.flags & IRSDE_FLAG_FP16) ? 1 : 0;
        } else if (!naive && (e->cfg.flags & (IRSDE_FLAG_SPLIT_BF16X2 | IRSDE_FLAG_SPLIT_F16X2)) && p.Cout >= 64 && p.nz == 1 && !p.ln_g &&
                   p.KH * p.KW * (p.C0 + p.C1) >= split_direct_min_k()) {
            const auto pc = e->pair_copy_il(p.w, (size_t)p.Cout, p.KH * p.KW * (p.C0 + p.C1));
            p.w_pair = pc.p; p.pair_scale = pc.inv_scale;
            p.f16 = (e->cfg.flags & IRSDE_FLAG_SPLIT_F16X2) ? 1 : 0;
        }
        Op op;
        op.kind = OP_CONV;
        op.flops = conv_flops(p);
        const double in_bytes = (p.in_bf16 || p.in_f16 ? 2.0 : 4.0) * (double)p.B * (p.Hin) * (p.Win) * (double)(p.C0 + p.C1);
        op.bytes = in_bytes + (p.out_bf16 || p.out_f16 ? 2.0 : 4.0) * (double)M * p.Cout +
                   (p.w_bf ? 2.0 : 4.0) * (double)p.Cout * p.KH * p.KW * (p.C0 + p.C1);
        op.exec_flops = op.flops;
        {
            long long launched = blocks;
            std::string kernel;
            if (!naive) {
                const ConvChoice c = conv_choose(p, ConvTune{}, conv_knobs_from_env(), device_cu_count());
                if (c.family == ConvChoice::HALO) kernel = conv_halo2_wanted(p) ? " kernel=halo512" : " kernel=halo256";
                else launched = c.blocks(), kernel = " kernel=" + c.name();
            }
            char buf[256];
            snprintf(buf, sizeof buf, "conv%s M=%d Cout=%d Cin=%d k=%dx%d s=%d up=%d splits=%d blocks=%lld flops=%.4g",
                     p.w_pair ? (p.f16 ? "(split f16x2)" : "(split bf16x2)") : p.w_bf ? (p.f16 ? (p.in_f16 || p.out_f16 ? "(fp16 operands + storage)" : "(fp16)") : "(bf16)") : "", M, p.Cout, p.C0 + p.C1, p.KH, p.KW, p.stride, p.in_shift, splits, launched, op.flops);
            op.desc = buf + kernel;
        }
        const bool nv = naive;
        op.fn = [p, nv](hipStream_t s) {
            if (nv)
                launch_conv_naive(p, s);
            else
                launch_conv(p, s);
        };
        push_op(std::move(op));
        if (p.partial) pl->release(p.partial);
    }

    Tensor conv(const ConvW& w, const Tensor& in0, const Tensor* in1, int stride, int pad, int in_shift,
                const float* film, int silu, const Tensor* res, int out_stride = 0) {
        ConvParams p;
        p.in0 = in0.p; p.C0 = in0.C; p.pix0 = in0.C;
        if (in1) { p.in1 = in1->p; p.C1 = in1->C; p.pix1 = in1->C; }
        if (p.C0 + p.C1 != w.Cin) throw HipError("conv: channel mismatch");
        p.Hin = in0.H; p.Win = in0.W; p.in_shift = in_shift;
        p.w = w.w; p.Cout = w.Cout; p.KH = w.KH; p.KW = w.KW; p.stride = stride; p.pad_y = pad; p.pad_x = pad;
        const int Hv = in0.H << in_shift, Wv = in0.W << in_shift;
        p.B = in0.B;
        p.Ho = (Hv + 2 * pad - w.KH) / stride + 1;
        p.Wo = (Wv + 2 * pad - w.KW) / stride + 1;
        const int ostr = out_stride ? out_stride : w.Cout;
        Tensor out = talloc(p.B, p.Ho, p.Wo, ostr, out_stride != 0);
        p.out = out.p; p.out_stride = ostr;
        p.in_bf16 = in0.bf16; p.out_bf16 = out.bf16;
        p.ln_g = fused_ln_g;
        if ((in1 && in1->bf16 != in0.bf16) || (res && res->bf16 != out.bf16)) throw HipError("conv: mixed activation storage types");
        p.bias = w.bias;
        p.film = film; p.film_bstride = film ? film_bstride : 0;
        p.silu = silu;
        if (res) { p.res = res->p; p.res_stride = res->C; }
        if (!naive) {
            if (w.wino_poly && push_wino_poly(p, w.wino_poly, w.wino_polyt)) return out;
            if (w.wino_up && wino_shape_ok(p, 4) && push_wino(p, w.wino_u4, 4, w.wino_up, w.wino_up_scale)) return out;
            if (split3_over_fused(w, p) && push_wino(p, w.wino_u4, 4, nullptr, 1.f, w.wino_u4t)) return out;
            if (w.wino_uf64p && push_wino_fused(p, reinterpret_cast<const float*>(w.wino_uf64p), true, w.wino_uf64p_scale)) return out;
            if (w.wino_uf64 && push_wino_fused(p, w.wino_uf64, true)) return out;
            if (w.wino_uf && push_wino_fused(p, w.wino_uf, false)) return out;
            if (w.wino_u4 && wino_shape_ok(p, 4) && push_wino(p, w.wino_u4, 4, nullptr, 1.f, w.wino_u4t)) return out;
            if (w.wino_u2 && wino_shape_ok(p, 2) && push_wino(p, w.wino_u2, 2)) return out;
        }
        push_conv(p);
        return out;
    }

    bool push_wino_fused(const ConvParams& d, const float* Uf, bool k64, float pair_uscale = 0.f) {
        ConvParams dd = d;
        dd.zeros = e->zeros;
        if (pair_uscale != 0.f) dd.pair_scale = 1.0f / (kWinoFused64PairVScale * pair_uscale);
        auto eligible = [&](const ConvParams& q) { return k64 ? wino_fused64_eligible(q) : wino_fused_eligible(q); };
        int parts = 1;
        if (!eligible(dd)) {
            for (parts = 2; parts <= 4; parts *= 2) {
                if (d.B % parts) continue;
                ConvParams q = dd;
                q.B = d.B / parts;
                if (eligible(q)) break;
            }
            if (parts > 4) return false;
            dd.B = d.B / parts;
        }
        const int Ctot = d.C0 + d.C1;
        const long long T = (long long)dd.B * (d.Ho / 4) * (d.Wo / 4);
        const long long blocks = k64 ? wino_fused64_num_blocks(dd) : (long long)dd.B * ((d.Ho / 4 + 3) / 4) * ((d.Wo / 4 + 7) / 8) * (d.Cout / 32);
        if (T < (k64 ? wino_fused64_min_tiles() : wino_fused_min_tiles()) || blocks < 256) return false;
        bool use_t = false;
        if (k64 && pair_uscale == 0.f && wino_fused64t_mode() && wino_fused64t_eligible(dd)) {
            const double per_block = (double)wino_fused64t_num_items(dd) / std::max(1, device_cu_count());
            const double work = per_block * (Ctot / 16);
            use_t = wino_fused64t_mode() >= 2 || (!d.in_shift && (work >= 64.0 || (work >= 32.0 && per_block >= 8.0 && !d.res)));
        }
        Op op;
        op.kind = OP_CONV;
        op.flops = conv_flops(d);
        op.exec_flops = 36 * 2.0 * (double)T * parts * Ctot * d.Cout;
        op.bytes = 4.0 * (double)d.B * d.Hin * d.Win * Ctot + 4.0 * (double)d.B * d.Ho * d.Wo * d.Cout + 4.0 * 9.0 * (double)d.Cout * Ctot;
        char buf[256];
        const bool pair = pair_uscale != 0.f;
        snprintf(buf, sizeof buf, "conv(%swinograd F4 fused) %s T=%lld Cout=%d Cin=%d up=%d blocks=%lld flops=%.4g exec=%.4g%s", pair ? "split f16x2 " : "",
                 use_t ? "32x64" : k64 ? "16x64" : "32x32", T * parts, d.Cout, Ctot, d.in_shift, blocks * parts, op.flops, op.exec_flops,
                 parts > 1 ? (parts == 2 ? " (2 batch slices)" : " (4 batch slices)") : "");
        op.desc = buf;
        std::vector<ConvParams> slices;
        for (int i = 0; i < parts; ++i) {
            ConvParams q = dd;
            const size_t b0 = (size_t)i * dd.B;
            q.in0 = dd.in0 + b0 * dd.Hin * dd.Win * dd.pix0;
            if (dd.in1) q.in1 = dd.in1 + b0 * dd.Hin * dd.Win * dd.pix1;
            q.out = dd.out + b0 * dd.Ho * dd.Wo * dd.out_stride;
            if (dd.res) q.res = dd.res + b0 * dd.Ho * dd.Wo * dd.res_stride;
            if (dd.film && dd.film_bstride) q.film = dd.film + b0 * dd.film_bstride;
            slices.push_back(q);
        }
        if (use_t)
            op.fn = [slices, Uf](hipStream_t s) { for (const auto& q : slices) launch_wino_fused64t(q, Uf, s, 0); };
        else if (k64)
            op.fn = [slices, Uf, pair](hipStream_t s) { for (const auto& q : slices) launch_wino_fused64(q, Uf, s, pair ? 4 : 0); };
        else
            op.fn = [slices, Uf](hipStream_t s) { for (const auto& q : slices) launch_wino_fused(q, Uf, s); };
        push_op(std::move(op));
        return true;
    }

    static constexpr long long kSplit3MinRows = 256;
    static constexpr int kSplit3MinCout = 512, kSplit3MinCoutPoly = 256;
    static constexpr double kSplit3MinFlop = 9e9;
    bool split3_rule(long long T, int K, int Cout, int ncomp, int min_cout = kSplit3MinCout) const {
        return T >= kSplit3MinRows && Cout >= min_cout && ncomp * 2.0 * (double)T * K * Cout >= kSplit3MinFlop;
    }
    bool split3_adopts(const unsigned short* Ut, long long T, int K, int Cout, int ncomp, int min_cout = kSplit3MinCout) const {
        const int mode = split3_mode();
        if (!Ut || mode <= 0 || naive || (e->cfg.flags & kSplit3NotExactF32) || !gemm_split_triples_fits(T, Cout, K, Cout)) return false;
        return mode >= 2 || split3_rule(T, K, Cout, ncomp, min_cout);
    }
    bool split3_over_fused(const ConvW& w, const ConvParams& p) const {
        if (!w.wino_u4t || p.C0 + p.C1 > 512 || !wino_shape_ok(p, 4)) return false;
        const long long T = (long long)p.B * (p.Ho / 4) * (p.Wo / 4);
        return T >= split3_fused_min_tiles() && split3_rule(T, p.C0 + p.C1, p.Cout, 36) && split3_adopts(w.wino_u4t, T, p.C0 + p.C1, p.Cout, 36);
    }
    static bool split3_attn_rule(int C, int N, int B) {
        (void)N; (void)B;
        return attn_split3_has_instance(C);
    }
// ... 703 lines not shown
    }
    b.tap("intro", x);
    const bool intro_skip = (e->cfg.flags & IRSDE_FLAG_NAF_INTRO_SKIP) != 0;
    const Tensor intro = x;
    auto run_level = [&](NafChainW& chain, const std::vector<NafBlockW>& blks, const std::string& path, int level) {
        auto advance = [&](const Tensor& y) {
            if (!(intro_skip && x.p == intro.p)) b.tfree(x);
            x = y;
        };
        if (!b.tlsc_local(x, level) && b.naf_chain_ok(chain, x))
            advance(b.nafchain(chain, x));
        else
            for (size_t j = 0; j < blks.size(); ++j) advance(block(blks[j], x, path + std::to_string(j), level));
    };
    std::vector<Tensor> encs;
    for (size_t i = 0; i < e->naf_enc.size(); ++i) {
        run_level(e->naf_chain_enc[i], e->naf_enc[i], "encoders." + std::to_string(i) + ".", (int)i);
        b.tap("encoders." + std::to_string(i), x);
        encs.push_back(x);
        Builder::ConvOpts od;
        od.stride = 2;
        x = b.conv_naf(e->naf_downs[i], x, od);
        b.tap("downs." + std::to_string(i), x);
    }
    const int nlev = (int)e->naf_enc.size();
    run_level(e->naf_chain_mid, e->naf_mid, "middle_blks.", nlev);
    b.tap("middle", x);
    for (size_t i = 0; i < e->naf_dec.size(); ++i) {
        Tensor skip = encs[encs.size() - 1 - i];
        Builder::ConvOpts ou;
        ou.shuffle = 1; ou.res = &skip;
        Tensor y = b.conv_naf(e->naf_ups[i], x, ou);
        b.tfree(x);
        b.tfree(skip);
        x = y;
        b.tap("ups." + std::to_string(i), x);
        run_level(e->naf_chain_dec[i], e->naf_dec[i], "decoders." + std::to_string(i) + ".", nlev - 1 - (int)i);
        b.tap("decoders." + std::to_string(i), x);
    }
    if (intro_skip) {
        Tensor y = b.talloc(x.B, x.H, x.W, x.C);
        const float *xa = x.p, *xb = intro.p;
        float* yo = y.p;
        const size_t n = x.numel();
        b.push_other(OP_OTHER, [=](hipStream_t s) { launch_add(xa, xb, yo, n, s); });
        b.tfree(x);
        b.tfree(intro);
        x = y;
    }
    Builder::ConvOpts oe;
    oe.pad = 1; oe.out_stride = stereo ? (e->naf_ic + 3) & ~3 : pl->pred_stride;
    Tensor pr = b.conv_naf(e->naf_ending, x, oe);
    b.tfree(x);
    if (stereo) {
        float* pred = pl->alloc((size_t)pl->B * pl->Hp * pl->Wp * pl->pred_stride, false);
        const float* src = pr.p;
        const int Bp = pl->B, ic = e->naf_ic, Hp = pl->Hp, Wp = pl->Wp, is = oe.out_stride, os = pl->pred_stride;
        b.push_other(OP_OTHER, [=](hipStream_t s) { launch_stereo_pack_pred(src, pred, Bp, ic, Hp, Wp, is, os, s); });
        pl->net_ops.back().desc = "stereo_pack_pred";
        pl->pred = pred;
        return;
    }
    pl->pred = pr.p;
}

static std::atomic<int> g_force_chain_groups{0};
void set_force_chain_groups(int g) { g_force_chain_groups.store(g, std::memory_order_relaxed); }
int forced_chain_groups() { return g_force_chain_groups.load(std::memory_order_relaxed); }
static std::atomic<int> g_force_scam_stream{0};
void set_force_scam_stream(int block_w) { g_force_scam_stream.store(block_w, std::memory_order_relaxed); }
int forced_scam_stream() { return g_force_scam_stream.load(std::memory_order_relaxed); }
static std::atomic<int> g_force_split3{-1};
void set_force_split3(int mode) { g_force_split3.store(mode, std::memory_order_relaxed); }
int split3_mode() {
    const int f = g_force_split3.load(std::memory_order_relaxed);
    return f >= 0 ? f : tuning_env_int("IRSDE_SPLIT3", 1);
}
static std::atomic<int> g_force_split3_attn{-1};
void set_force_split3_attn(int mode) { g_force_split3_attn.store(mode, std::memory_order_relaxed); }
int split3_attn_mode() {
    const int f = g_force_split3_attn.load(std::memory_order_relaxed);
    return f >= 0 ? f : tuning_env_int("IRSDE_SPLIT3_ATTN", 1);
}
static std::atomic<int> g_force_wino_poly{-1};
void set_force_wino_poly(int mode) { g_force_wino_poly.store(mode, std::memory_order_relaxed); }
int wino_poly_mode() {
    const int f = g_force_wino_poly.load(std::memory_order_relaxed);
    return f >= 0 ? f : tuning_env_int("IRSDE_WINO_POLY", 1);
}
static std::atomic<int> g_force_subbatches{0};
void set_force_subbatches(int n) { g_force_subbatches.store(n, std::memory_order_relaxed); }
int naf_subbatches(const irsde_engine* e, int B, int H, int W) {
    if (e->arch == 2 || stereo_engine(e) || (e->cfg.flags & (IRSDE_FLAG_NAIVE_CONV | IRSDE_FLAG_KEEP_ACTIVATIONS))) return 1;
    int n = g_force_subbatches.load(std::memory_order_relaxed);
    if (n <= 0) {
        static const int env = tuning_env_int("IRSDE_SUBBATCHES", 0);
        n = env;
    }
    if (n <= 0 && e->arch != 1) n = 1;
    if (n <= 0) {
        bool chain = false;
        const int nlev = (int)e->naf_enc.size(), ps = 1 << nlev;
        const int Hp = (H + ps - 1) / ps * ps, Wp = (W + ps - 1) / ps * ps;
        if ((e->cfg.flags & IRSDE_FLAG_FP16) && !(e->cfg.flags & (IRSDE_FLAG_NO_NAF_CHAIN | IRSDE_FLAG_F16_ACT)))
            for (int i = 0; i < nlev; ++i)
                if (e->naf_chain_enc[i].nblocks > 0 && naf_chain_shape_ok(Hp >> i, Wp >> i, e->naf_intro.Cout << i)) {
                    int K0 = 0, K1 = 0;
                    if (!tlsc_window(e, i, &K0, &K1) || (K0 >= (Hp >> i) && K1 >= (Wp >> i))) chain = true;
                }
        n = chain && B >= 8 ? 2 : 1;
    }
    n = std::min(n, (int)irsde_engine::kMaxSub);
    while (n > 1 && B % n) --n;
    return std::max(n, 1);
}

static bool evict_lru_plan(irsde_engine* e) {
    if (e->plans.empty()) return false;
    size_t lru = 0;
    for (size_t i = 1; i < e->plans.size(); ++i)
        if (e->plans[i]->last_use < e->plans[lru]->last_use) lru = i;
    IRSDE_HIP_CHECK(hipDeviceSynchronize());
    const int vb = e->plans[lru]->B, vh = e->plans[lru]->H, vw = e->plans[lru]->W;
    const bool split = e->plans[lru]->slot > 0;
    for (size_t i = e->plans.size(); i-- > 0;)
        if (i == lru || (split && e->plans[i]->slot > 0 && e->plans[i]->B == vb && e->plans[i]->H == vh && e->plans[i]->W == vw))
            e->plans.erase(e->plans.begin() + i);
    return true;
}

static Plan* build_plan(irsde_engine* e, int B, int H, int W, bool per_sample_film, int slot, int b0);

static void init_plan_geometry(irsde_engine* e, Plan* pl, int B, int H, int W, int sdiv) {
    pl->B = B; pl->H = H; pl->W = W;
    pl->Hp = (H + sdiv - 1) / sdiv * sdiv;
    pl->Wp = (W + sdiv - 1) / sdiv * sdiv;
    pl->last_use = ++e->use_counter;
    if (e->arch != 1 && (pl->Hp - H >= H || pl->Wp - W >= W)) throw HipError("image too small for reflect padding");
}

Plan* get_plan(irsde_engine* e, int B, int H, int W, bool per_sample_film, int slot, int b0) {
    for (auto& p : e->plans)
        if (p->B == B && p->H == H && p->W == W && p->per_sample_film == per_sample_film && p->slot == slot && p->b0 == b0) {
            p->last_use = ++e->use_counter;
            return p.get();
        }
    if (e->plans.size() >= 8) evict_lru_plan(e);
    for (;;) {
        try {
            return build_plan(e, B, H, W, per_sample_film, slot, b0);
        } catch (const HipOutOfMemory&) {
            if (!evict_lru_plan(e)) throw;
        }
    }
}

static Plan* build_plan(irsde_engine* e, int B, int H, int W, bool per_sample_film, int slot, int b0) {
    const bool stereo = stereo_engine(e), ustereo = unet_stereo(e);
    if (stereo && slot > 0) throw HipError("internal: a stereo batch is never split into sub-batches");
    ensure_film_cur(e, per_sample_film ? (stereo ? 2 : 1) * (b0 + B) : 1);
    if (naf_lens(e)) {
        if (e->cam_set < b0 + B) throw HipError("latent-bokeh ConditionalNAFNet: irsde_set_lens_info must cover the batch first");
        if (e->cam_rows < b0 + B) throw HipError("internal: lens table smaller than the batch");
    }

    const int depth = e->cfg.depth, nf = e->cfg.nf, in_nc = e->cfg.in_nc;
// ... 236 lines not shown
```

### image_restoration_sde_amd/csrc/gemm_split.hip

```cpp
#include "common.h"
#include <algorithm>
#include <atomic>
#include <type_traits>

namespace irsde {

typedef float floatx16 __attribute__((ext_vector_type(16)));
typedef __bf16 bf16x8 __attribute__((ext_vector_type(8)));
typedef _Float16 f16x8 __attribute__((ext_vector_type(8)));
typedef unsigned uintx4 __attribute__((ext_vector_type(4)));

namespace {

constexpr int SG_BK = 32;

#define IRSDE_GLDS16(GPTR, LPTR) \
    __builtin_amdgcn_global_load_lds((const __attribute__((address_space(1))) void*)(GPTR), (__attribute__((address_space(3))) void*)(LPTR), 16, 0, 0)

template <int ABL = 0, bool F16 = false>
__global__ __launch_bounds__(512, 2) void gemm_split2i_kernel(const SplitGemmArgs g) {
    using frag_t = typename std::conditional<F16, f16x8, bf16x8>::type;
    constexpr int TM = 4, TN = 2, WN = 4, BM = 256, BN = 256;
    constexpr int A_STAGE = BM * 128, STAGE = (BM + BN) * 128;
    extern __shared__ __attribute__((aligned(16))) char lds[];
    const int tid = threadIdx.x, lane = tid & 63;
    const int wave = __builtin_amdgcn_readfirstlane(tid >> 6);
    const int wm = wave / WN, wn = wave % WN;
    const int l31 = lane & 31, h = lane >> 5;
    const int mtiles = (g.M + BM - 1) / BM;
    const int units = mtiles * g.n_inner;
    const int xcd = blockIdx.x & 7, jx = blockIdx.x >> 3;
    const int ulo = (int)((long long)xcd * units / 8), uhi = (int)((long long)(xcd + 1) * units / 8);
    const int unit = ulo + jx / g.nblk_n;
    if (unit >= uhi) return;
    const int nblk = jx % g.nblk_n;
    const int plane0 = unit / mtiles, mblk = unit - plane0 * mtiles;
    const int m0 = mblk * BM, n0 = nblk * BN;
    const int nk = g.K / SG_BK;
    const int steps = nk;
    const unsigned rowb = (unsigned)nk * 128u;

    unsigned a_voff[4], b_voff[4];
#pragma unroll
    for (int ps = 0; ps < 4; ++ps) {
        const int row = (ps * 8 + wave) * 8 + (lane >> 3);
        const unsigned pc = (unsigned)((lane & 7) ^ ((row >> 1) & 7)) * 16u;
        int m = m0 + row;
        m = m < g.M ? m : g.M - 1;
        a_voff[ps] = (unsigned)m * rowb + pc;
        int n = n0 + row;
        n = n < g.N ? n : g.N - 1;
        b_voff[ps] = (unsigned)n * rowb + pc;
    }
    const char* abase = reinterpret_cast<const char*>(g.a);
    const char* bbase = reinterpret_cast<const char*>(g.b);
    const long long pA2 = g.pA * 4, pB2 = g.pB * 4;
    int kb = 0;
    const char* acomp = abase + (long long)plane0 * pA2;
    const char* bcomp = bbase + (long long)plane0 * pB2;
    auto issue_loads = [&](int buf) {
        char* la = lds + buf * STAGE + wave * 1024;
        const char* ga = acomp + kb * 128;
        const char* gb = bcomp + kb * 128;
#pragma unroll
        for (int ps = 0; ps < 4; ++ps) IRSDE_GLDS16(ga + a_voff[ps], la + ps * 8192);
#pragma unroll
        for (int ps = 0; ps < 4; ++ps) IRSDE_GLDS16(gb + b_voff[ps], la + A_STAGE + ps * 8192);
    };

    auto issue_loads_part = [&](int buf, int part) {
        char* la = lds + buf * STAGE + wave * 1024;
        const char* ga = acomp + kb * 128;
        const char* gb = bcomp + kb * 128;
        if (part == 0) {
            IRSDE_GLDS16(ga + a_voff[0], la);
            IRSDE_GLDS16(ga + a_voff[1], la + 8192);
            IRSDE_GLDS16(ga + a_voff[2], la + 2 * 8192);
        } else if (part == 1) {
            IRSDE_GLDS16(ga + a_voff[3], la + 3 * 8192);
            IRSDE_GLDS16(gb + b_voff[0], la + A_STAGE);
            IRSDE_GLDS16(gb + b_voff[1], la + A_STAGE + 8192);
        } else {
            IRSDE_GLDS16(gb + b_voff[2], la + A_STAGE + 2 * 8192);
            IRSDE_GLDS16(gb + b_voff[3], la + A_STAGE + 3 * 8192);
        }
    };

    floatx16 acc[TM][TN];
#pragma unroll
    for (int i = 0; i < TM; ++i)
#pragma unroll
        for (int j = 0; j < TN; ++j)
#pragma unroll
// ... 187 lines not shown
        read_b(0, lds + b_base);
        __builtin_amdgcn_sched_barrier(0);
        for (int st = 0; st < nk; ++st) {
            const bool more1 = st + 1 < nk, more2 = st + 2 < nk;
            const char* a = lds + (st & 1) * STAGE + a_base;
            const char* b = lds + (st & 1) * STAGE + b_base;
            const char* an = lds + ((st + 1) & 1) * STAGE + a_base;
            const char* bn = lds + ((st + 1) & 1) * STAGE + b_base;
#pragma unroll
            for (int i = 0; i < TM; ++i) {
                if (i == 1) {
                    read_a(0, a + 32 * ROWB);
                    __builtin_amdgcn_sched_barrier(0);
                }
#pragma unroll
                for (int sb = 0; sb < 2; ++sb)
#pragma unroll
                    for (int pr = 0; pr < 6; ++pr) {
#pragma unroll
                        for (int j = 0; j < TN; ++j) {
                            if (ABL != 3) acc[i][j] = __builtin_amdgcn_mfma_f32_32x32x16_bf16(fa[sb][PA[pr]], fb[sb][PB[pr]][j], acc[i][j], 0, 0, 0);
                            else acc[i][j][0] += (float)fa[sb][PA[pr]][0] * (float)fb[sb][PB[pr]][j][0];
                        }
                        __builtin_amdgcn_sched_barrier(0);
                        if (sb == 0 && pr == 0) {
                            if (i == 0) {
                                read_a(1, a);
                                read_b(1, b);
                            } else {
                                read_a(1, a + 32 * ROWB);
                            }
                        }
                        if (i == 1 && sb == 1 && pr == 0 && more1) {
                            read_a(0, an);
                            read_b(0, bn);
                        }
                        if (ABL != 1 && (sb == 1) == late) {
                            if (i == 0 && pr >= 1 && pr <= 3 && more1) issue_one(st + 1, 1, pr - 1);
                            if (i == 1 && more2) issue_one(st + 2, pr < 3 ? 0 : 2, pr % 3);
                        }
                        __builtin_amdgcn_sched_barrier(0);
                    }
                if (DRAIN || (i == 0 && !more1)) IRSDE_WAIT_VM(0);
                else if (i == 0) IRSDE_WAIT_VM(3);
                IRSDE_PHASE_BARRIER();
            }
        }

        const int rowb_ = m0 + wm * TM * 32, colb = n0 + wn * TN * 32;
        float* ob = g.out + (long long)plane0 * g.pO + (long long)rowb_ * g.ldc;
        const int rows = g.M - rowb_;
        const unsigned nrec = rows <= 0 ? 0u : (unsigned)(rows < TM * 32 ? rows : TM * 32) * (unsigned)g.ldc * 4u;
        const __amdgpu_buffer_rsrc_t ro = __builtin_amdgcn_make_buffer_rsrc(ob, 0, nrec, 0x00020000);
        it += it_step;
        const bool next = WALK && it < nitems;
        if (next) {
            set_item(it);
            issue_first();
            __builtin_amdgcn_sched_barrier(0);
        }
#pragma unroll
        for (int i = 0; i < TM; ++i)
#pragma unroll
            for (int j = 0; j < TN; ++j) {
                const int colu = colb + j * 32;
                if (colu + l31 < g.N && (ABL != 4 || acc[i][j][0] == 1.2345e30f)) {
#pragma unroll
                    for (int r = 0; r < 16; ++r) {
                        const float v = acc[i][j][r];
                        const unsigned voff = (unsigned)((i * 32 + (r & 3) + 8 * (r >> 2) + 4 * h) * g.ldc + colu + l31) * 4u;
                        __builtin_amdgcn_raw_buffer_store_b32(__builtin_bit_cast(unsigned, v), ro, (int)voff, 0, 0);
                    }
                }
            }
        if (!next) break;
#pragma unroll
        for (int i = 0; i < TM; ++i)
#pragma unroll
            for (int j = 0; j < TN; ++j)
#pragma unroll
                for (int r = 0; r < 16; ++r) acc[i][j][r] = 0.f;
    }
}
#undef IRSDE_PHASE_BARRIER
#undef IRSDE_WAIT_VM
#undef IRSDE_GLDS16

__global__ __launch_bounds__(256) void split_triples_kernel(const float* __restrict__ in, unsigned short* __restrict__ out, const size_t n, const size_t rows,
                                                            const int K) {
    const size_t i = (size_t)blockIdx.x * blockDim.x + threadIdx.x;
    if (i >= n) return;
    const size_t rk = rows * (size_t)K;
    const size_t z = i / rk, rem = i - z * rk;
    const size_t row = rem / K;
    const int k = (int)(rem - row * K);
    float r = in[i];
    unsigned short* o = out + z * split3_comp_elems(rows, K);
#pragma unroll
    for (int p = 0; p < 3; ++p) {
        const __bf16 hb = (__bf16)r;
        o[split3_index(row, k, p, K / 32)] = __builtin_bit_cast(unsigned short, hb);
        r -= (float)hb;
    }
}

template <bool F16>
__global__ __launch_bounds__(256) void split_pairs_kernel(const float* __restrict__ in, unsigned short* __restrict__ out, const size_t n, const int K,
                                                          const float scale) {
    const size_t i = (size_t)blockIdx.x * blockDim.x + threadIdx.x;
    if (i >= n) return;
    const size_t row = i / K;
    const int k = (int)(i - row * K);
    float r = in[i];
    const size_t base = (row * (size_t)(K / 32) + k / 32) * 64 + (k & 31);
    if constexpr (F16) {
        r *= scale;
        const _Float16 hb = (_Float16)r;
        out[base] = __builtin_bit_cast(unsigned short, hb);
        r -= (float)hb;
        const _Float16 lb = (_Float16)r;
        out[base + 32] = __builtin_bit_cast(unsigned short, lb);
    } else {
        const __bf16 hb = (__bf16)r;
        out[base] = __builtin_bit_cast(unsigned short, hb);
        r -= (float)hb;
        const __bf16 lb = (__bf16)r;
        out[base + 32] = __builtin_bit_cast(unsigned short, lb);
    }
}

template <int NPL, bool F16 = false>
__global__ __launch_bounds__(256) void split_planes_kernel(const float* __restrict__ in, unsigned short* __restrict__ out, const size_t n,
                                                           const size_t plane, const float scale) {
    const size_t i = (size_t)blockIdx.x * blockDim.x + threadIdx.x;
    if (i >= n) return;
    float r = F16 ? in[i] * scale : in[i];
#pragma unroll
    for (int p = 0; p < NPL; ++p) {
        if constexpr (F16) {
            const _Float16 hb = (_Float16)r;
            out[p * plane + i] = __builtin_bit_cast(unsigned short, hb);
            r -= (float)hb;
        } else {
            const __bf16 hb = (__bf16)r;
            out[p * plane + i] = __builtin_bit_cast(unsigned short, hb);
            r -= (float)hb;
        }
    }
}

__global__ __launch_bounds__(256) void split_frag3_kernel(const float* __restrict__ in, unsigned short* __restrict__ out, const size_t n, const int K) {
    const size_t i = (size_t)blockIdx.x * blockDim.x + threadIdx.x;
    if (i >= n) return;
    const size_t row = i / K;
    const int k = (int)(i - row * K);
    float r = in[i];
    const size_t o = attn_frag3_index(row, k, K);
#pragma unroll
    for (int p = 0; p < 3; ++p) {
        const __bf16 hb = (__bf16)r;
        out[p * n + o] = __builtin_bit_cast(unsigned short, hb);
        r -= (float)hb;
    }
}

}

void launch_split_frag3(const float* in, unsigned short* out, size_t rows, int K, hipStream_t s) {
    if (rows % 32 || K % 16) throw HipError("split_frag3: rows must be a multiple of 32, K of 16");
    const size_t n = rows * (size_t)K;
    hipLaunchKernelGGL(split_frag3_kernel, dim3((unsigned)((n + 255) / 256)), dim3(256), 0, s, in, out, n, K);
    IRSDE_HIP_CHECK(hipGetLastError());
}

void gemm_split_global_init() {
    IRSDE_HIP_CHECK(hipFuncSetAttribute(reinterpret_cast<const void*>(gemm_split2i_kernel<0>), hipFuncAttributeMaxDynamicSharedMemorySize, 160 * 1024));
    IRSDE_HIP_CHECK(hipFuncSetAttribute(reinterpret_cast<const void*>(gemm_split2i_kernel<0, true>), hipFuncAttributeMaxDynamicSharedMemorySize, 160 * 1024));
    IRSDE_HIP_CHECK(hipFuncSetAttribute(reinterpret_cast<const void*>(gemm_split2i_kernel<5, true>), hipFuncAttributeMaxDynamicSharedMemorySize, 160 * 1024));
    IRSDE_HIP_CHECK(hipFuncSetAttribute(reinterpret_cast<const void*>(gemm_split2i_kernel<1>), hipFuncAttributeMaxDynamicSharedMemorySize, 160 * 1024));
    IRSDE_HIP_CHECK(hipFuncSetAttribute(reinterpret_cast<const void*>(gemm_split2i_kernel<3>), hipFuncAttributeMaxDynamicSharedMemorySize, 160 * 1024));
    IRSDE_HIP_CHECK(hipFuncSetAttribute(reinterpret_cast<const void*>(gemm_split2i_kernel<4>), hipFuncAttributeMaxDynamicSharedMemorySize, 160 * 1024));
    IRSDE_HIP_CHECK(hipFuncSetAttribute(reinterpret_cast<const void*>(gemm_split3i_kernel<0, true>), hipFuncAttributeMaxDynamicSharedMemorySize, 160 * 1024));
    IRSDE_HIP_CHECK(hipFuncSetAttribute(reinterpret_cast<const void*>(gemm_split3i_kernel<0, false>), hipFuncAttributeMaxDynamicSharedMemorySize, 160 * 1024));
    IRSDE_HIP_CHECK(hipFuncSetAttribute(reinterpret_cast<const void*>(gemm_split3i_kernel<0, true, true>), hipFuncAttributeMaxDynamicSharedMemorySize, 160 * 1024));
#ifdef IRSDE_PROBES
    IRSDE_HIP_CHECK(hipFuncSetAttribute(reinterpret_cast<const void*>(gemm_split3i_kernel<1, true>), hipFuncAttributeMaxDynamicSharedMemorySize, 160 * 1024));
    IRSDE_HIP_CHECK(hipFuncSetAttribute(reinterpret_cast<const void*>(gemm_split3i_kernel<3, true>), hipFuncAttributeMaxDynamicSharedMemorySize, 160 * 1024));
    IRSDE_HIP_CHECK(hipFuncSetAttribute(reinterpret_cast<const void*>(gemm_split3i_kernel<4, true>), hipFuncAttributeMaxDynamicSharedMemorySize, 160 * 1024));
    IRSDE_HIP_CHECK(hipFuncSetAttribute(reinterpret_cast<const void*>(gemm_split3i_kernel<1, false>), hipFuncAttributeMaxDynamicSharedMemorySize, 160 * 1024));
    IRSDE_HIP_CHECK(hipFuncSetAttribute(reinterpret_cast<const void*>(gemm_split3i_kernel<3, false>), hipFuncAttributeMaxDynamicSharedMemorySize, 160 * 1024));
    IRSDE_HIP_CHECK(hipFuncSetAttribute(reinterpret_cast<const void*>(gemm_split3i_kernel<4, false>), hipFuncAttributeMaxDynamicSharedMemorySize, 160 * 1024));
    IRSDE_HIP_CHECK(hipFuncSetAttribute(reinterpret_cast<const void*>(gemm_split3i_kernel<1, true, true>), hipFuncAttributeMaxDynamicSharedMemorySize, 160 * 1024));
    IRSDE_HIP_CHECK(hipFuncSetAttribute(reinterpret_cast<const void*>(gemm_split3i_kernel<3, true, true>), hipFuncAttributeMaxDynamicSharedMemorySize, 160 * 1024));
    IRSDE_HIP_CHECK(hipFuncSetAttribute(reinterpret_cast<const void*>(gemm_split3i_kernel<4, true, true>), hipFuncAttributeMaxDynamicSharedMemorySize, 160 * 1024));
#endif
}

void launch_gemm_split_pairs(const SplitGemmArgs& a, int ncomp, hipStream_t s, int abl, bool f16) {
    if (a.K % SG_BK) throw HipError("gemm_split_pairs: K must be a multiple of 32");
    if ((unsigned long long)a.M * a.K * 4ull >= 0xffffffffull || (unsigned long long)a.N * a.K * 4ull >= 0xffffffffull ||
        (size_t)a.M * a.ldc * 4 >= 0xffffffffull)
        throw HipError("gemm_split_pairs: a component exceeds the 32-bit offset range");
    SplitGemmArgs g = a;
    g.nblk_n = (a.N + 255) / 256;
    g.n_inner = ncomp;
    const int units = ((a.M + 255) / 256) * ncomp;
    int per_xcd = 0;
    for (int x = 0; x < 8; ++x) per_xcd = std::max(per_xcd, (int)((long long)(x + 1) * units / 8) - (int)((long long)x * units / 8));
    const dim3 grid((unsigned)(8 * per_xcd * g.nblk_n));
    const size_t lds = (size_t)2 * 512 * 128;
    if (f16) {
        if (abl != 0) throw HipError("gemm_split_pairs: the ablation twins exist for the bf16 kernel only");
        static const bool nt = tuning_env_int("IRSDE_SPLIT_NT", 0) != 0;
        if (nt) hipLaunchKernelGGL((gemm_split2i_kernel<5, true>), grid, dim3(512), lds, s, g);
        else hipLaunchKernelGGL((gemm_split2i_kernel<0, true>), grid, dim3(512), lds, s, g);
        IRSDE_HIP_CHECK(hipGetLastError());
        return;
    }
    switch (abl) {
        case 0: hipLaunchKernelGGL(gemm_split2i_kernel<0>, grid, dim3(512), lds, s, g); break;
        case 1: hipLaunchKernelGGL(gemm_split2i_kernel<1>, grid, dim3(512), lds, s, g); break;
        case 3: hipLaunchKernelGGL(gemm_split2i_kernel<3>, grid, dim3(512), lds, s, g); break;
        case 4: hipLaunchKernelGGL(gemm_split2i_kernel<4>, grid, dim3(512), lds, s, g); break;
        default: throw HipError("gemm_split_pairs: bad ablation variant");
    }
    IRSDE_HIP_CHECK(hipGetLastError());
}

bool gemm_split_triples_fits(long long M, long long N, long long K, long long ldc) {
    if (M < 1 || N < 1 || K < 32 || K % SG_BK) return false;
    return (unsigned long long)split3_comp_elems((size_t)M, (size_t)K) * 2ull < 0xffffffffull && (unsigned long long)split3_comp_elems((size_t)N, (size_t)K) * 2ull < 0xffffffffull &&
           (unsigned long long)M * ldc * 4ull < 0xffffffffull;
}

static std::atomic<int> g_force_split3_blocks{-1};
void set_force_split3_blocks(int n) { g_force_split3_blocks.store(n >= 8 ? n : -1, std::memory_order_relaxed); }

template <int ABL>
static void launch_split3_abl(bool walk, bool drain, dim3 grid, size_t lds, hipStream_t s, const SplitGemmArgs& g) {
    if (drain) hipLaunchKernelGGL((gemm_split3i_kernel<ABL, true, true>), grid, dim3(512), lds, s, g);
    else if (walk) hipLaunchKernelGGL((gemm_split3i_kernel<ABL, true>), grid, dim3(512), lds, s, g);
    else hipLaunchKernelGGL((gemm_split3i_kernel<ABL, false>), grid, dim3(512), lds, s, g);
}
void launch_gemm_split_triples(const SplitGemmArgs& a, int ncomp, hipStream_t s, const Split3Launch& o) {
    if (a.K % SG_BK) throw HipError("gemm_split_triples: K must be a multiple of 32");
    if (!gemm_split_triples_fits(a.M, a.N, a.K, a.ldc)) throw HipError("gemm_split_triples: a component exceeds the 32-bit offset range");
    if (ncomp < 1 || a.ldc < a.N) throw HipError("gemm_split_triples: bad component count or output stride");
    static const bool walk_knob = tuning_env_int("IRSDE_SPLIT3_WALK", 1) != 0, drain_knob = tuning_env_int("IRSDE_SPLIT3_DRAIN", 0) != 0;
    const bool walk = o.walk == Split3Launch::RULE ? walk_knob : o.walk == Split3Launch::ON;
    const bool drain = o.drain == Split3Launch::RULE ? drain_knob : o.drain == Split3Launch::ON;
    if (drain && !walk) throw HipError("gemm_split_triples: the drain twin exists on the walk only");
    SplitGemmArgs g = a;
    g.nblk_n = (a.N + 127) / 128;
    g.n_inner = ncomp;
    const long long units = (long long)((a.M + 255) / 256) * ncomp;
    long long per_xcd = 0;
    for (int x = 0; x < 8; ++x) per_xcd = std::max(per_xcd, (x + 1) * units / 8 - x * units / 8);
    long long blocks = 8 * per_xcd * g.nblk_n;
    if (blocks >= 0x7fffffffll) throw HipError("gemm_split_triples: grid too large");
    if (walk) {
        const int forced = g_force_split3_blocks.load(std::memory_order_relaxed);
        blocks = std::min<long long>(blocks, std::max(8, forced > 0 ? forced : device_cu_count()));
    }
    const dim3 grid((unsigned)blocks);
    const size_t lds = (size_t)2 * (256 + 128) * 192;
    switch (o.abl) {
        case Split3Launch::FULL: launch_split3_abl<0>(walk, drain, grid, lds, s, g); break;
#ifdef IRSDE_PROBES
        case Split3Launch::NO_LOADS: launch_split3_abl<1>(walk, drain, grid, lds, s, g); break;
        case Split3Launch::NO_MFMA: launch_split3_abl<3>(walk, drain, grid, lds, s, g); break;
        case Split3Launch::NO_STORES: launch_split3_abl<4>(walk, drain, grid, lds, s, g); break;
#endif
        default: throw HipError("gemm_split_triples: the ablation twins are part of the PROBES build");
    }
    IRSDE_HIP_CHECK(hipGetLastError());
}

void launch_split_triples(const float* in, unsigned short* out, int ncomp, size_t rows, int K, hipStream_t s) {
    if (K % 32 || ncomp < 1 || rows < 1) throw HipError("split_triples: K must be a multiple of 32");
    const size_t n = (size_t)ncomp * rows * (size_t)K;
    hipLaunchKernelGGL(split_triples_kernel, dim3((unsigned)((n + 255) / 256)), dim3(256), 0, s, in, out, n, rows, K);
    IRSDE_HIP_CHECK(hipGetLastError());
}

void launch_split_pairs(const float* in, unsigned short* out, size_t rows, int K, hipStream_t s, bool f16, float scale) {
    if (K % 32) throw HipError("split_pairs: K must be a multiple of 32");
    const size_t n = rows * (size_t)K;
    if (f16) hipLaunchKernelGGL(split_pairs_kernel<true>, dim3((unsigned)((n + 255) / 256)), dim3(256), 0, s, in, out, n, K, scale);
    else hipLaunchKernelGGL(split_pairs_kernel<false>, dim3((unsigned)((n + 255) / 256)), dim3(256), 0, s, in, out, n, K, 1.0f);
    IRSDE_HIP_CHECK(hipGetLastError());
}

void launch_split_planes(const float* in, unsigned short* out, size_t n, size_t plane, int nplanes, hipStream_t s, bool f16, float scale) {
    const dim3 grid((unsigned)((n + 255) / 256));
    if (f16 && nplanes != 2) throw HipError("split_planes: fp16 pieces come in pairs");
    if (f16) hipLaunchKernelGGL((split_planes_kernel<2, true>), grid, dim3(256), 0, s, in, out, n, plane, scale);
    else if (nplanes == 2) hipLaunchKernelGGL((split_planes_kernel<2, false>), grid, dim3(256), 0, s, in, out, n, plane, 1.0f);
    else throw HipError("split_planes: 2 planes");
    IRSDE_HIP_CHECK(hipGetLastError());
}

}
```

### include/irsde_hip_debug.h

```cpp
#ifndef IRSDE_HIP_DEBUG_H
#define IRSDE_HIP_DEBUG_H

#include "irsde_hip.h"

#ifdef __cplusplus
extern "C" {
#endif

int irsde_debug_conv(const float* in0, int C0, const float* in1, int C1, int B, int Hin, int Win, int in_shift,
                     const float* w_oihw, int Cout, int KH, int KW, int stride, int pad, const float* bias,
                     const float* film, int film_bstride, int silu, const float* res, float* out, int naive,
                     int splits, void* stream);

int irsde_debug_conv_choice(int B, int Hin, int Win, int C0, int C1, int Cout, int K, int stride, int pad, int in_shift, int operand, int storage, int pair,
                            unsigned features, int splits, int nz, int tune, int cu_count, const int* knobs, char* out, int out_len);

int irsde_debug_conv_halo_choice(int B, int Hin, int Win, int C0, int C1, int Cout, int K, int stride, int pad, int in_shift, int operand, int storage, int pair,
                                 unsigned features, int splits, int nz, int tune, int halo2, int nslow, char* out, int out_len);

int irsde_debug_conv_features(const float* in0, int C0, const float* in1, int C1, int B, int Hin, int Win, int in_shift, const float* w_oihw, int Cout, int K,
                              int stride, int pad, int operand, int storage, int pair, const float* bias, const float* ch_scale, const float* ln_g,
                              const float* film, int film_bstride, const float* res, const float* in_scale, const float* gate_film, int gate_film_bstride,
                              int silu, int gate, int shuffle, int nz, int splits, int tune, const int* knobs, float* out, char* choice, int choice_len,
                              void* stream);

int irsde_debug_split_gemm(const float* A, const float* B, float* C, int M, int N, int K, int ncomp, int nplanes, void* stream);

int irsde_bench_conv(int variant, int B, int H, int W, int Cin, int Cout, int K, int stride, int up, int epi, int iters,
                     double* ms_out);
int irsde_bench_naf_chain(int variant, int nblocks, int B, int iters, double* ms_out);
int irsde_debug_force_subbatches(int n);
int irsde_debug_force_chain_groups(int g);
int irsde_debug_force_wino_poly(int mode);
int irsde_debug_force_split3(int mode);
int irsde_debug_force_split3_attn(int mode);
int irsde_debug_force_split3_blocks(int n);

int irsde_debug_scam(const float* x, int B_pairs, int H, int W, int C, const float* norm_l_g, const float* norm_r_g, const float* l_proj1_w,
                     const float* l_proj1_b, const float* r_proj1_w, const float* r_proj1_b, const float* l_proj2_w, const float* l_proj2_b,
                     const float* r_proj2_w, const float* r_proj2_b, const float* beta, const float* gamma, float* out, void* stream);

int irsde_debug_naf_gate_sca(const float* u, int B, int H, int W, int c, const float* conv2_w, const float* conv2_b, const float* sca_w, const float* sca_b,
                             float* gated_out, float* mean_out, float* s_out, void* stream);
int irsde_debug_tlsc(const float* g, int B, int h, int w, int c, int k1, int k2, float* pooled_out, const float* scale_map, float* scaled_out, void* stream);
int irsde_debug_ln_film(const float* x, long long M, int C, long long ppi, const float* g, const float* fscale, const float* fshift, int film_bstride,
                        float* out, void* stream);
int irsde_debug_naf_lnconv(int mode, const float* x, long long M, int c, int Cout, long long ppi, const float* g, const float* fscale, const float* fshift,
                           int film_bstride, const float* w, const float* bias, const float* gate_film, int gate_film_bstride, const float* in_scale,
                           const float* ch_scale, const float* res, float* out, void* stream);

int irsde_debug_naf_chain(const float* x, float* out, int B, int nblocks, const float* norm1_g, const float* conv1_w, const float* conv1_b, const float* conv2_w,
                          const float* conv2_b, const float* sca_w, const float* sca_b, const float* conv3_w, const float* conv3_b, const float* beta,
                          const float* norm2_g, const float* conv4_w, const float* conv4_b, const float* conv5_w, const float* conv5_b, const float* gamma,
                          const float* film, int film_bstride, int film_off, const float* cam, int cam_bstride, int cam_off, int groups, void* stream);
int irsde_debug_naf_chain_split_order(int nblocks, int groups, int* order_out, long long n);

int irsde_debug_full_attention16(const void* qkv_bf16, int B, int N, void* out_bf16, void* stream);

int irsde_debug_scam_full(const float* x, int B_pairs, int H, int W, int C, const float* norm_l_g, const float* norm_r_g, const float* l_proj1_w,
                          const float* l_proj1_b, const float* r_proj1_w, const float* r_proj1_b, const float* l_proj2_w, const float* l_proj2_b,
                          const float* r_proj2_w, const float* r_proj2_b, const float* beta, const float* gamma, float* out, void* stream);

int irsde_debug_scam_stream(const float* x, int B_pairs, int H, int W, int C, const float* norm_l_g, const float* norm_r_g, const float* l_proj1_w,
                            const float* l_proj1_b, const float* r_proj1_w, const float* r_proj1_b, const float* l_proj2_w, const float* l_proj2_b,
                            const float* r_proj2_w, const float* r_proj2_b, const float* beta, const float* gamma, int block_w, float* out, void* stream);
int irsde_debug_scam_full_stream(const float* x, int B_pairs, int H, int W, int C, const float* norm_l_g, const float* norm_r_g, const float* l_proj1_w,
                                 const float* l_proj1_b, const float* r_proj1_w, const float* r_proj1_b, const float* l_proj2_w, const float* l_proj2_b,
                                 const float* r_proj2_w, const float* r_proj2_b, const float* beta, const float* gamma, int block_w, float* out,
                                 void* stream);
int irsde_debug_force_scam_stream(int block_w);

#ifdef __cplusplus
}
#endif
#endif
```

Baseline: 4.999 images/s.

## Route eligible plain 1x1 convolutions through a bf16x3 split MFMA GEMM kernel

Adds a persistent bf16x3 split-precision GEMM kernel (256x128 tiles, 512 threads, double-buffered LDS) for plain 1x1 convolutions. The kernel reads fp32 activations directly, with an optional two-input concat, and uses pre-split row-pair weight triples cached per layer. The planner adopts it by default for large 1x1 layers without epilogues, in place of the generic fp32 conv path, to get matrix-core throughput while keeping near-fp32 accuracy. In exchange it does roughly three times the MFMA work and adds weight-copy memory. Its benefit depends on how much of the time the 1x1 layers take in this UNet.

```diff
diff --git a/image_restoration_sde_amd/_lib.py b/image_restoration_sde_amd/_lib.py
--- a/image_restoration_sde_amd/_lib.py
+++ b/image_restoration_sde_amd/_lib.py
@@ -39,7 +39,7 @@
     "irsde_last_error", "irsde_version", "irsde_create", "irsde_create_nafnet", "irsde_destroy", "irsde_num_weights",
     "irsde_weight_name", "irsde_weight_shape", "irsde_load_weight", "irsde_finalize_weights",
     "irsde_set_schedule", "irsde_unet_forward", "irsde_sample", "irsde_sde_step", "irsde_philox_normal",
-    "irsde_get_profile", "irsde_debug_tap", "irsde_work_model", "irsde_debug_conv", "irsde_debug_conv_choice", "irsde_debug_conv_halo_choice", "irsde_debug_conv_features", "irsde_plan_describe", "irsde_bench_conv", "irsde_op_profile", "irsde_debug_split_gemm", "irsde_bench_naf_chain", "irsde_debug_force_subbatches", "irsde_debug_force_chain_groups", "irsde_debug_force_wino_poly", "irsde_debug_force_split3", "irsde_debug_force_split3_attn", "irsde_debug_force_split3_blocks", "irsde_debug_scam", "irsde_debug_scam_full",
+    "irsde_get_profile", "irsde_debug_tap", "irsde_work_model", "irsde_debug_conv", "irsde_debug_conv_choice", "irsde_debug_conv_halo_choice", "irsde_debug_conv_features", "irsde_plan_describe", "irsde_bench_conv", "irsde_op_profile", "irsde_debug_split_gemm", "irsde_bench_naf_chain", "irsde_debug_force_subbatches", "irsde_debug_force_chain_groups", "irsde_debug_force_wino_poly", "irsde_debug_force_split3", "irsde_debug_force_split3_attn", "irsde_debug_force_split3_blocks", "irsde_debug_force_split3_1x1", "irsde_debug_split3_1x1", "irsde_debug_split3_1x1_choice", "irsde_debug_scam", "irsde_debug_scam_full",
     "irsde_debug_scam_stream", "irsde_debug_scam_full_stream", "irsde_debug_force_scam_stream",
     "irsde_debug_naf_gate_sca", "irsde_debug_tlsc", "irsde_debug_ln_film", "irsde_debug_naf_lnconv", "irsde_debug_naf_chain", "irsde_debug_naf_chain_split_order",
     "irsde_debug_full_attention16",
@@ -133,6 +133,9 @@
     lib.irsde_debug_force_wino_poly.argtypes = [c.c_int]
     lib.irsde_debug_force_split3.argtypes = [c.c_int]
     lib.irsde_debug_force_split3_attn.argtypes = [c.c_int]
+    lib.irsde_debug_force_split3_1x1.argtypes = [c.c_int]
+    lib.irsde_debug_split3_1x1.argtypes = [P, c.c_int, c.c_int, P, c.c_int, c.c_int, P, P, P, c.c_int, c.c_int, c.c_int, c.c_int, P]
+    lib.irsde_debug_split3_1x1_choice.argtypes = [c.c_int] * 13 + [c.c_uint] + [c.c_int] * 6 + [c.c_char_p, c.c_int]
     lib.irsde_debug_force_split3_blocks.argtypes = [c.c_int]
     lib.irsde_debug_scam.argtypes = [P, c.c_int, c.c_int, c.c_int, c.c_int] + [P] * 12 + [P, P]
     lib.irsde_debug_scam_full.argtypes = [P, c.c_int, c.c_int, c.c_int, c.c_int] + [P] * 12 + [P, P]
diff --git a/image_restoration_sde_amd/csrc/common.h b/image_restoration_sde_amd/csrc/common.h
--- a/image_restoration_sde_amd/csrc/common.h
+++ b/image_restoration_sde_amd/csrc/common.h
@@ -141,6 +141,28 @@
 void set_force_split3_blocks(int n);
 bool gemm_split_triples_fits(long long M, long long N, long long K, long long ldc);
 void launch_split_triples(const float* in, unsigned short* out, int ncomp, size_t rows, int K, hipStream_t s);
+struct Split3aArgs {
+    const float* in0 = nullptr;
+    const float* in1 = nullptr;
+    int C0 = 0, C1 = 0;
+    int pix0 = 0, pix1 = 0;
+    const unsigned short* w3 = nullptr;
+    const float* bias = nullptr;
+    float* out = nullptr;
+    int M = 0, N = 0, out_stride = 0;
+    int nblk_n = 0;
+};
+bool gemm_split3a_fits(const Split3aArgs& a, const char** why_not = nullptr);
+int gemm_split3a_blocks(long long M, int N, int cus, bool walk = true);
+constexpr size_t kSplit3aLds = (size_t)2 * (256 * 128 + 128 * 192);
+void launch_gemm_split3a(const Split3aArgs& a, hipStream_t s, const Split3Launch& o = {});
+struct Split3x1Choice {
+    bool adopt = false;
+    const char* why_not = "";
+    int grid = 0, lds = 0;
+};
+Split3x1Choice split3_1x1_choose(const ConvParams& p, bool exact_f32, int master, int knob, int cus);
+Split3aArgs split3_1x1_args(const ConvParams& p, const unsigned short* w3);
 void launch_split_planes(const float* in, unsigned short* out, size_t n, size_t plane, int nplanes, hipStream_t s, bool f16 = false,
                          float scale = 1.0f);
 void launch_wino_output(const WinoParams& p, hipStream_t s);
diff --git a/image_restoration_sde_amd/csrc/engine.h b/image_restoration_sde_amd/csrc/engine.h
--- a/image_restoration_sde_amd/csrc/engine.h
+++ b/image_restoration_sde_amd/csrc/engine.h
@@ -7,6 +7,7 @@
 #include <memory>
 #include <mutex>
 #include <string>
+#include <tuple>
 #include <vector>
 
 #include "../../include/irsde_hip.h"
@@ -41,6 +42,8 @@
 inline bool split3_wants_weights(int flags) { return !(flags & kSplit3NotExactF32) && split3_mode() > 0; }
 int split3_attn_mode();
 void set_force_split3_attn(int mode);
+int split3_1x1_mode();
+void set_force_split3_1x1(int mode);
 
 inline int wino_min_c(int tile) {
     return tuning_env_int(tile == 4 ? "IRSDE_WINO4_MINC" : "IRSDE_WINO2_MINC", tile == 4 ? 64 : 256);
@@ -433,17 +436,20 @@
     PairCopy pair_copy(const float* w, size_t n) {
         return make_pair_copy(pair_copies, w, n, [&](unsigned short* d, bool f16, float sc) { launch_split_planes(w, d, n, n, 2, stream, f16, sc); });
     }
-    std::map<const float*, unsigned short*> triple_copies;
-    const unsigned short* triple_copy(const float* w, size_t rows, int K) {
-        const size_t n = rows * (size_t)K;
-        auto it = triple_copies.find(w);
+    enum TripleLayout { TRIPLES_FRAG3 = 0, TRIPLES_ROWPAIR = 1 };
+    std::map<std::tuple<const float*, int, size_t>, unsigned short*> triple_copies;
+    const unsigned short* triple_copy(const float* w, size_t rows, int K, TripleLayout layout = TRIPLES_FRAG3) {
+        const auto key = std::make_tuple(w, (int)layout, rows);
+        auto it = triple_copies.find(key);
         if (it != triple_copies.end()) return it->second;
+        const size_t elems = layout == TRIPLES_ROWPAIR ? split3_comp_elems(rows, (size_t)K) : 3 * rows * (size_t)K;
         unsigned short* d = nullptr;
-        IRSDE_HIP_CHECK(hipMalloc(&d, 3 * n * sizeof(unsigned short)));
+        IRSDE_HIP_CHECK(hipMalloc(&d, elems * sizeof(unsigned short)));
         dev_allocs.push_back(reinterpret_cast<float*>(d));
-        launch_split_frag3(w, d, rows, K, stream);
+        if (layout == TRIPLES_ROWPAIR) launch_split_triples(w, d, 1, rows, K, stream);
+        else launch_split_frag3(w, d, rows, K, stream);
         IRSDE_HIP_CHECK(hipStreamSynchronize(stream));
-        triple_copies[w] = d;
+        triple_copies[key] = d;
         return d;
     }
     std::map<const float*, PairCopy> pair_copies_il;
diff --git a/image_restoration_sde_amd/csrc/engine_debug.hip b/image_restoration_sde_amd/csrc/engine_debug.hip
--- a/image_restoration_sde_amd/csrc/engine_debug.hip
+++ b/image_restoration_sde_amd/csrc/engine_debug.hip
@@ -110,6 +110,7 @@
     Fused64,
     Fused64Pair,
     Fused64T,
+    Split3a,
 };
 struct DebugConvRow {
     int code;
@@ -133,7 +134,7 @@
     wino(3, ConvPath::WinoF4, 0), wino(13, ConvPath::WinoF4, 71), wino(23, ConvPath::WinoF4, 72),
     poly(24, ConvPath::Poly, false), poly(25, ConvPath::Poly, true),
     poly(26, ConvPath::PolyTriples, false), poly(27, ConvPath::PolyTriples, true), poly(28, ConvPath::PolyTriples, true, true),
-    on_path(48, ConvPath::F4Triples),
+    on_path(48, ConvPath::F4Triples), on_path(49, ConvPath::Split3a),
     on_path(44, ConvPath::F4Pairs, Operand::F16), on_path(45, ConvPath::F4Pairs, Operand::BF16),
     on_path(46, ConvPath::DirectPair, Operand::F16), on_path(47, ConvPath::DirectPair, Operand::BF16),
     on_path(33, ConvPath::Fused32),
@@ -162,6 +163,7 @@
     Fused64TStamps,
     PairGemm,
     TripleGemm,
+    Split3aGemm,
 };
 struct BenchRow {
     int lo, hi;
@@ -198,6 +200,7 @@
     bench(4650, 4653, BenchKind::Fused64TStamps, 12),
     bench(472, 476, BenchKind::PairGemm, 0),
     bench(490, 504, BenchKind::TripleGemm, 0),
+    bench(510, 524, BenchKind::Split3aGemm, 0),
 };
 
 template <class Row, size_t N, class Lo, class Hi>
@@ -670,6 +673,15 @@
             launch_wino_output(sp.out, s);
             break;
         }
+        case ConvPath::Split3a: {
+            if (splits > 1) p.splits = splits;
+            const Split3x1Choice c = split3_1x1_choose(p, true, 2, 2, device_cu_count());
+            if (!c.adopt) throw HipError(std::string("debug_conv: selector 49 runs a plain 1x1 layer (bias only): ") + c.why_not);
+            unsigned short* dwt = mem.alloc<unsigned short>(split3_comp_elems((size_t)Cout, (size_t)Cin));
+            launch_split_triples(dw, dwt, 1, (size_t)Cout, Cin, s);
+            launch_gemm_split3a(split3_1x1_args(p, dwt), s);
+            break;
+        }
         case ConvPath::F4Pairs: {
             const bool f16 = r.op == Operand::F16;
             if (!wino_shape_ok(p, 4) || Cin % 32) throw HipError("debug_conv: shape not eligible for the pair GEMM");
@@ -948,6 +960,42 @@
     set_force_split3_attn(mode >= 0 && mode <= 2 ? mode : -1);
     return IRSDE_OK;
 }
+int irsde_debug_force_split3_1x1(int mode) {
+    set_force_split3_1x1(mode >= 0 && mode <= 2 ? mode : -1);
+    return IRSDE_OK;
+}
+
+int irsde_debug_split3_1x1(const float* in0, int C0, int pix0, const float* in1, int C1, int pix1, const float* w, const float* bias, float* out, int M, int N,
+                           int out_stride, int mode, void* stream) {
+    return guard([&] {
+        if (!in0 || !w || !out || (C1 && !in1) || mode < 0 || mode > 2) throw HipError("debug_split3_1x1: bad argument");
+        hipStream_t s = reinterpret_cast<hipStream_t>(stream);
+        conv_global_init();
+        Split3aArgs a;
+        a.in0 = in0; a.C0 = C0; a.pix0 = pix0; a.in1 = C1 ? in1 : nullptr; a.C1 = C1; a.pix1 = C1 ? pix1 : 0;
+        a.bias = bias; a.out = out; a.M = M; a.N = N; a.out_stride = out_stride;
+        const char* why = nullptr;
+        if (!gemm_split3a_fits(a, &why)) throw HipError(std::string("debug_split3_1x1: ") + why);
+        Scratch mem(s);
+        unsigned short* wt = mem.alloc<unsigned short>(split3_comp_elems((size_t)N, (size_t)(C0 + C1)));
+        launch_split_triples(w, wt, 1, (size_t)N, C0 + C1, s);
+        a.w3 = wt;
+        launch_gemm_split3a(a, s, split3_launch_twin(mode));
+        IRSDE_HIP_CHECK(hipStreamSynchronize(s));
+    });
+}
+
+int irsde_debug_split3_1x1_choice(int B, int Hin, int Win, int C0, int C1, int Cout, int K, int stride, int pad, int in_shift, int operand, int storage, int pair,
+                                  unsigned features, int splits, int nz, int engine_flags, int master, int knob, int cu_count, char* out, int out_len) {
+    return guard([&] {
+        if (!out || out_len < 1 || K < 1 || stride < 1 || cu_count < 1 || operand < 0 || operand > 2 || storage < 0 || storage > 2 || (pair && operand == 0))
+            throw HipError("debug_split3_1x1_choice: bad argument");
+        const ConvParams p = choice_hook_params(B, Hin, Win, C0, C1, Cout, K, stride, pad, in_shift, operand, storage, pair, features, splits, nz);
+        const Split3x1Choice c = split3_1x1_choose(p, !(engine_flags & kSplit3NotExactF32), master, knob, cu_count);
+        snprintf(out, (size_t)out_len, "adopt=%d grid=%d lds=%d why_not=%s", c.adopt ? 1 : 0, c.grid, c.lds, c.why_not);
+    });
+}
+
 int irsde_debug_force_split3_blocks(int n) {
     if (n >= 0 && n < 8) return guard([&] { throw HipError("debug_force_split3_blocks: n must be at least 8 (one block per XCD), or negative for the default"); });
     set_force_split3_blocks(n);
@@ -1113,6 +1161,17 @@
             unsigned short* dwp = mem.alloc<unsigned short>(2 * nw);
             launch_split_pairs(dw, dwp, (size_t)Cout, K * K * Cin, s, f16, 64.0f);
             p.w_pair = dwp; p.pair_scale = 1.0f / 64.0f; p.f16 = f16 ? 1 : 0;
+        }
+        if (kind == BenchKind::Split3aGemm) {
+            const Split3x1Choice c = split3_1x1_choose(p, true, 2, 2, device_cu_count());
+            if (!c.adopt || up || epi) throw HipError(std::string("bench_conv: variants 510 - 524 run a plain 1x1 layer: ") + (c.adopt ? "no epilogue" : c.why_not));
+            unsigned short* dwt = mem.alloc<unsigned short>(split3_comp_elems((size_t)Cout, (size_t)Cin));
+            launch_split_triples(dw, dwt, 1, (size_t)Cout, Cin, s);
+            const Split3aArgs a = split3_1x1_args(p, dwt);
+            const Split3Launch twin = split3_launch_twin(arg / 5, arg % 5);
+            for (int i = 0; i < 2; ++i) launch_gemm_split3a(a, s, twin);
+            *ms_out = time_launches(s, iters, [&] { launch_gemm_split3a(a, s, twin); });
+            return;
         }
         if (kind == BenchKind::TripleGemm || kind == BenchKind::PairGemm) {
             if (K != 3 || stride != 1 || !wino_shape_ok(p, 4)) throw HipError("bench_conv: Winograd variants need an eligible 3x3 stride-1 layer");
diff --git a/image_restoration_sde_amd/csrc/engine_plan.hip b/image_restoration_sde_amd/csrc/engine_plan.hip
--- a/image_restoration_sde_amd/csrc/engine_plan.hip
+++ b/image_restoration_sde_amd/csrc/engine_plan.hip
@@ -38,7 +38,7 @@
         pl->net_ops.push_back(std::move(op));
     }
 
-    void push_conv(ConvParams p) {
+    int conv_splits(const ConvParams& p) const {
         const int M = p.B * p.Ho * p.Wo;
         const int bn = conv_base_bn(p.Cout);
         const int blocks = ((M + 127) / 128) * ((p.Cout + bn - 1) / bn);
@@ -48,6 +48,35 @@
             splits = std::min(std::min(nk / 8, (512 + blocks - 1) / blocks), 16);
             if (splits < 2) splits = 1;
         }
+        return splits;
+    }
+
+    bool push_split3_1x1(const ConvParams& p0) {
+        if (p0.KH != 1 || p0.KW != 1 || naive) return false;
+        ConvParams p = p0;
+        p.splits = conv_splits(p);
+        const Split3x1Choice c = split3_1x1_choose(p, !(e->cfg.flags & kSplit3NotExactF32), split3_mode(), split3_1x1_mode(), device_cu_count());
+        if (!c.adopt) return false;
+        const int M = p.B * p.Ho * p.Wo, K = p.C0 + p.C1;
+        const Split3aArgs a = split3_1x1_args(p, e->triple_copy(p.w, (size_t)p.Cout, K, irsde_engine::TRIPLES_ROWPAIR));
+        Op op;
+        op.kind = OP_CONV;
+        op.flops = conv_flops(p);
+        op.exec_flops = op.flops;
+        op.bytes = 4.0 * (double)p.B * p.Hin * p.Win * (double)K + 4.0 * (double)M * p.Cout + 4.0 * (double)p.Cout * K;
+        char buf[256];
+        snprintf(buf, sizeof buf, "conv M=%d Cout=%d Cin=%d k=%dx%d s=%d up=%d splits=%d blocks=%d flops=%.4g kernel=split3a bf16x3", M, p.Cout, K, p.KH, p.KW,
+                 p.stride, p.in_shift, 1, c.grid, op.flops);
+        op.desc = buf;
+        op.fn = [a](hipStream_t s) { launch_gemm_split3a(a, s); };
+        push_op(std::move(op));
+        return true;
+    }
+
+    void push_conv(ConvParams p) {
+        const int M = p.B * p.Ho * p.Wo;
+        const int blocks = ((M + 127) / 128) * ((p.Cout + conv_base_bn(p.Cout) - 1) / conv_base_bn(p.Cout));
+        const int splits = conv_splits(p);
         if (splits > 1) {
             p.splits = splits;
             p.partial = pl->alloc((size_t)splits * M * p.Cout, true);
@@ -124,6 +153,7 @@
             if (w.wino_uf && push_wino_fused(p, w.wino_uf, false)) return out;
             if (w.wino_u4 && wino_shape_ok(p, 4) && push_wino(p, w.wino_u4, 4, nullptr, 1.f, w.wino_u4t)) return out;
             if (w.wino_u2 && wino_shape_ok(p, 2) && push_wino(p, w.wino_u2, 2)) return out;
+            if (push_split3_1x1(p)) return out;
         }
         push_conv(p);
         return out;
@@ -993,6 +1023,12 @@
     const int f = g_force_split3_attn.load(std::memory_order_relaxed);
     return f >= 0 ? f : tuning_env_int("IRSDE_SPLIT3_ATTN", 1);
 }
+static std::atomic<int> g_force_split3_1x1{-1};
+void set_force_split3_1x1(int mode) { g_force_split3_1x1.store(mode, std::memory_order_relaxed); }
+int split3_1x1_mode() {
+    const int f = g_force_split3_1x1.load(std::memory_order_relaxed);
+    return f >= 0 ? f : tuning_env_int("IRSDE_SPLIT3_1X1", 1);
+}
 static std::atomic<int> g_force_wino_poly{-1};
 void set_force_wino_poly(int mode) { g_force_wino_poly.store(mode, std::memory_order_relaxed); }
 int wino_poly_mode() {
diff --git a/image_restoration_sde_amd/csrc/gemm_split.hip b/image_restoration_sde_amd/csrc/gemm_split.hip
--- a/image_restoration_sde_amd/csrc/gemm_split.hip
+++ b/image_restoration_sde_amd/csrc/gemm_split.hip
@@ -9,6 +9,7 @@
 typedef __bf16 bf16x8 __attribute__((ext_vector_type(8)));
 typedef _Float16 f16x8 __attribute__((ext_vector_type(8)));
 typedef unsigned uintx4 __attribute__((ext_vector_type(4)));
+typedef float floatx4 __attribute__((ext_vector_type(4)));
 
 namespace {
 
@@ -362,6 +363,229 @@
                 for (int r = 0; r < 16; ++r) acc[i][j][r] = 0.f;
     }
 }
+template <int ABL = 0, bool WALK = true, bool DRAIN = false>
+__global__ __launch_bounds__(512, 1) void gemm_split3a_kernel(const Split3aArgs g) {
+    constexpr int TN = 4, BM = 256, BN = 128;
+    constexpr int AROW = 128, BROW = 192;
+    constexpr int A_STAGE = BM * AROW, B_HALF = 64 * BROW, STAGE = A_STAGE + 2 * B_HALF;
+    constexpr int PA[6] = {0, 1, 2, 0, 1, 0};
+    constexpr int PB[6] = {2, 1, 0, 1, 0, 0};
+    extern __shared__ __attribute__((aligned(16))) char lds[];
+    const int tid = threadIdx.x, lane = tid & 63;
+    const int wave = __builtin_amdgcn_readfirstlane(tid >> 6);
+    const int l31 = lane & 31, h = lane >> 5;
+    const int units = (g.M + BM - 1) / BM;
+    const int xcd = blockIdx.x & 7, jx = blockIdx.x >> 3;
+    const int ulo = (int)((long long)xcd * units / 8), uhi = (int)((long long)(xcd + 1) * units / 8);
+    const int nitems = (uhi - ulo) * g.nblk_n;
+    const int it_step = WALK ? ((int)gridDim.x - xcd + 7) >> 3 : nitems;
+    int it = jx;
+    if (it >= nitems) return;
+    const int nk0 = g.C0 / SG_BK, nk = (g.C0 + g.C1) / SG_BK;
+    const unsigned pairb = (unsigned)nk * 384u;
+
+    int m0, n0;
+    unsigned a_voff0[4], a_voff1[4], b_voff[2][2];
+    float bias_r[TN];
+    auto set_item = [&](int i) {
+        const int unit = ulo + i / g.nblk_n, nblk = i % g.nblk_n;
+        m0 = unit * BM;
+        n0 = nblk * BN;
+#pragma unroll
+        for (int ps = 0; ps < 4; ++ps) {
+            const int row = (ps * 8 + wave) * 8 + (lane >> 3);
+            const unsigned pc = (unsigned)((lane & 7) ^ ((row >> 1) & 7)) * 16u;
+            int m = m0 + row;
+            m = m < g.M ? m : g.M - 1;
+            a_voff0[ps] = (unsigned)m * (unsigned)g.pix0 * 4u + pc;
+            a_voff1[ps] = (unsigned)m * (unsigned)g.pix1 * 4u + pc;
+        }
+#pragma unroll
+        for (int hb = 0; hb < 2; ++hb)
+#pragma unroll
+            for (int wl = 0; wl < 2; ++wl) {
+                const int sl = wl * 32 + lane;
+                const int r = sl / 12, pos = sl - r * 12;
+                const int rowt = wave * 8 + r;
+                int j = pos - ((rowt >> 2) & 3);
+                j = j < 0 ? j + 12 : j;
+                int n = n0 + hb * 64 + rowt;
+                n = n < g.N ? n : g.N - 1;
+                b_voff[hb][wl] = (unsigned)(n >> 1) * pairb + (unsigned)(n & 1) * 192u + (unsigned)j * 16u;
+            }
+        if (g.bias) {
+#pragma unroll
+            for (int j = 0; j < TN; ++j) {
+                int n = n0 + j * 32 + l31;
+                n = n < g.N ? n : g.N - 1;
+                bias_r[j] = g.bias[n];
+            }
+        }
+    };
+    auto issue_a = [&](int kb, int ps) {
+        const bool second = kb >= nk0;
+        const char* gsrc = second ? reinterpret_cast<const char*>(g.in1) + (size_t)(kb - nk0) * 128 : reinterpret_cast<const char*>(g.in0) + (size_t)kb * 128;
+        IRSDE_GLDS16(gsrc + (second ? a_voff1[ps] : a_voff0[ps]), lds + (kb & 1) * STAGE + (ps * 8 + wave) * 1024);
+    };
+    auto issue_b = [&](int kb, int hb, int wl) {
+        const char* gsrc = reinterpret_cast<const char*>(g.w3) + (size_t)kb * 384;
+        IRSDE_GLDS16(gsrc + b_voff[hb][wl], lds + (kb & 1) * STAGE + A_STAGE + hb * B_HALF + wave * 8 * BROW + wl * 512);
+    };
+    auto issue_first = [&]() {
+        issue_b(0, 0, 0); issue_b(0, 0, 1);
+#pragma unroll
+        for (int ps = 0; ps < 4; ++ps) issue_a(0, ps);
+        issue_b(0, 1, 0); issue_b(0, 1, 1);
+        if (nk > 1) {
+#pragma unroll
+            for (int ps = 0; ps < 4; ++ps) issue_a(1, ps);
+            issue_b(1, 0, 0); issue_b(1, 0, 1);
+        }
+    };
+
+    floatx16 acc[TN];
+#pragma unroll
+    for (int j = 0; j < TN; ++j)
+#pragma unroll
+        for (int r = 0; r < 16; ++r) acc[j][r] = 0.f;
+
+    set_item(it);
+    issue_first();
+
+    const int swz = (l31 >> 1) & 7;
+    int fa_off[2][2], fr_off[3][2];
+#pragma unroll
+    for (int sb = 0; sb < 2; ++sb)
+#pragma unroll
+        for (int e = 0; e < 2; ++e) fa_off[sb][e] = l31 * AROW + (((2 * (2 * sb + h) + e) ^ swz) * 16);
+#pragma unroll
+    for (int p = 0; p < 3; ++p)
+#pragma unroll
+        for (int sb = 0; sb < 2; ++sb) fr_off[p][sb] = l31 * BROW + ((p * 4 + sb * 2 + h + ((l31 >> 2) & 3)) % 12) * 16;
+    bf16x8 fa[2][3], fb[2][3][2];
+    floatx4 ra[2];
+    auto read_a = [&](int sb, const char* a) {
+#pragma unroll
+        for (int e = 0; e < 2; ++e) ra[e] = *reinterpret_cast<const floatx4*>(a + fa_off[sb][e]);
+    };
+    auto split_a = [&](int sb) {
+#pragma unroll
+        for (int e = 0; e < 8; ++e) {
+            float r = ra[e >> 2][e & 3];
+#pragma unroll
+            for (int p = 0; p < 3; ++p) {
+                const __bf16 hb = (__bf16)r;
+                fa[sb][p][e] = hb;
+                r -= (float)hb;
+            }
+        }
+    };
+    auto read_b = [&](int sb, const char* b) {
+#pragma unroll
+        for (int p = 0; p < 3; ++p)
+#pragma unroll
+            for (int j = 0; j < 2; ++j) fb[sb][p][j] = *reinterpret_cast<const bf16x8*>(b + j * 32 * BROW + fr_off[p][sb]);
+    };
+    const bool late = wave >= 4;
+    const int a_base = wave * 32 * AROW;
+    for (;;) {
+        IRSDE_WAIT_VM(0);
+        IRSDE_PHASE_BARRIER();
+        read_a(0, lds + a_base);
+        read_b(0, lds + A_STAGE);
+        split_a(0);
+        __builtin_amdgcn_sched_barrier(0);
+        for (int st = 0; st < nk; ++st) {
+            const bool more1 = st + 1 < nk, more2 = st + 2 < nk;
+            const char* a = lds + (st & 1) * STAGE + a_base;
+            const char* b = lds + (st & 1) * STAGE + A_STAGE;
+            const char* an = lds + ((st + 1) & 1) * STAGE + a_base;
+            const char* bn = lds + ((st + 1) & 1) * STAGE + A_STAGE;
+#pragma unroll
+            for (int i = 0; i < 2; ++i) {
+                if (i == 1) {
+                    read_b(0, b + B_HALF);
+                    __builtin_amdgcn_sched_barrier(0);
+                }
+#pragma unroll
+                for (int sb = 0; sb < 2; ++sb)
+#pragma unroll
+                    for (int pr = 0; pr < 6; ++pr) {
+#pragma unroll
+                        for (int j = 0; j < 2; ++j) {
+                            if (ABL != 3) acc[2 * i + j] = __builtin_amdgcn_mfma_f32_32x32x16_bf16(fa[sb][PA[pr]], fb[sb][PB[pr]][j], acc[2 * i + j], 0, 0, 0);
+                            else acc[2 * i + j][0] += (float)fa[sb][PA[pr]][0] * (float)fb[sb][PB[pr]][j][0];
+                        }
+                        __builtin_amdgcn_sched_barrier(0);
+                        if (sb == 0 && pr == 0) {
+                            if (i == 0) {
+                                read_a(1, a);
+                                read_b(1, b);
+                            } else {
+                                read_b(1, b + B_HALF);
+                            }
+                        }
+                        if (i == 0 && sb == 0 && pr == 3) split_a(1);
+                        if (i == 1 && sb == 1 && more1) {
+                            if (pr == 0) {
+                                read_a(0, an);
+                                read_b(0, bn);
+                            }
+                            if (pr == 3) split_a(0);
+                        }
+                        if (ABL != 1 && (sb == 1) == late) {
+                            if (i == 0 && pr >= 1 && pr <= 2 && more1) issue_b(st + 1, 1, pr - 1);
+                            if (i == 1 && more2) {
+                                if (pr < 4) issue_a(st + 2, pr);
+                                else issue_b(st + 2, 0, pr - 4);
+                            }
+                        }
+                        __builtin_amdgcn_sched_barrier(0);
+                    }
+                if (DRAIN || (i == 0 && !more1)) IRSDE_WAIT_VM(0);
+                else if (i == 0) IRSDE_WAIT_VM(2);
+                IRSDE_PHASE_BARRIER();
+            }
+        }
+
+        if (g.bias) {
+#pragma unroll
+            for (int j = 0; j < TN; ++j)
+#pragma unroll
+                for (int r = 0; r < 16; ++r) acc[j][r] += bias_r[j];
+        }
+        const int rowb_ = m0 + wave * 32, colb = n0;
+        float* ob = g.out + (long long)rowb_ * g.out_stride;
+        const int rows = g.M - rowb_;
+        const unsigned nrec = rows <= 0 ? 0u : (unsigned)(rows < 32 ? rows : 32) * (unsigned)g.out_stride * 4u;
+        const __amdgpu_buffer_rsrc_t ro = __builtin_amdgcn_make_buffer_rsrc(ob, 0, nrec, 0x00020000);
+        it += it_step;
+        const bool next = WALK && it < nitems;
+        if (next) {
+            __builtin_amdgcn_sched_barrier(0);
+            set_item(it);
+            issue_first();
+            __builtin_amdgcn_sched_barrier(0);
+        }
+#pragma unroll
+        for (int j = 0; j < TN; ++j) {
+            const int colu = colb + j * 32;
+            if (colu + l31 < g.N && (ABL != 4 || acc[j][0] == 1.2345e30f)) {
+#pragma unroll
+                for (int r = 0; r < 16; ++r) {
+                    const float v = acc[j][r];
+                    const unsigned voff = (unsigned)(((r & 3) + 8 * (r >> 2) + 4 * h) * g.out_stride + colu + l31) * 4u;
+                    __builtin_amdgcn_raw_buffer_store_b32(__builtin_bit_cast(unsigned, v), ro, (int)voff, 0, 0);
+                }
+            }
+        }
+        if (!next) break;
+#pragma unroll
+        for (int j = 0; j < TN; ++j)
+#pragma unroll
+            for (int r = 0; r < 16; ++r) acc[j][r] = 0.f;
+    }
+}
 #undef IRSDE_PHASE_BARRIER
 #undef IRSDE_WAIT_VM
 #undef IRSDE_GLDS16
@@ -463,7 +687,16 @@
     IRSDE_HIP_CHECK(hipFuncSetAttribute(reinterpret_cast<const void*>(gemm_split3i_kernel<0, true>), hipFuncAttributeMaxDynamicSharedMemorySize, 160 * 1024));
     IRSDE_HIP_CHECK(hipFuncSetAttribute(reinterpret_cast<const void*>(gemm_split3i_kernel<0, false>), hipFuncAttributeMaxDynamicSharedMemorySize, 160 * 1024));
     IRSDE_HIP_CHECK(hipFuncSetAttribute(reinterpret_cast<const void*>(gemm_split3i_kernel<0, true, true>), hipFuncAttributeMaxDynamicSharedMemorySize, 160 * 1024));
+    IRSDE_HIP_CHECK(hipFuncSetAttribute(reinterpret_cast<const void*>(gemm_split3a_kernel<0, true>), hipFuncAttributeMaxDynamicSharedMemorySize, 160 * 1024));
+    IRSDE_HIP_CHECK(hipFuncSetAttribute(reinterpret_cast<const void*>(gemm_split3a_kernel<0, false>), hipFuncAttributeMaxDynamicSharedMemorySize, 160 * 1024));
+    IRSDE_HIP_CHECK(hipFuncSetAttribute(reinterpret_cast<const void*>(gemm_split3a_kernel<0, true, true>), hipFuncAttributeMaxDynamicSharedMemorySize, 160 * 1024));
 #ifdef IRSDE_PROBES
+    for (const void* f : {reinterpret_cast<const void*>(gemm_split3a_kernel<1, true>), reinterpret_cast<const void*>(gemm_split3a_kernel<3, true>),
+                          reinterpret_cast<const void*>(gemm_split3a_kernel<4, true>), reinterpret_cast<const void*>(gemm_split3a_kernel<1, false>),
+                          reinterpret_cast<const void*>(gemm_split3a_kernel<3, false>), reinterpret_cast<const void*>(gemm_split3a_kernel<4, false>),
+                          reinterpret_cast<const void*>(gemm_split3a_kernel<1, true, true>), reinterpret_cast<const void*>(gemm_split3a_kernel<3, true, true>),
+                          reinterpret_cast<const void*>(gemm_split3a_kernel<4, true, true>)})
+        IRSDE_HIP_CHECK(hipFuncSetAttribute(f, hipFuncAttributeMaxDynamicSharedMemorySize, 160 * 1024));
     IRSDE_HIP_CHECK(hipFuncSetAttribute(reinterpret_cast<const void*>(gemm_split3i_kernel<1, true>), hipFuncAttributeMaxDynamicSharedMemorySize, 160 * 1024));
     IRSDE_HIP_CHECK(hipFuncSetAttribute(reinterpret_cast<const void*>(gemm_split3i_kernel<3, true>), hipFuncAttributeMaxDynamicSharedMemorySize, 160 * 1024));
     IRSDE_HIP_CHECK(hipFuncSetAttribute(reinterpret_cast<const void*>(gemm_split3i_kernel<4, true>), hipFuncAttributeMaxDynamicSharedMemorySize, 160 * 1024));
@@ -556,6 +789,114 @@
     IRSDE_HIP_CHECK(hipGetLastError());
 }
 
+bool gemm_split3a_fits(const Split3aArgs& a, const char** why_not) {
+    const char* why = nullptr;
+    const unsigned long long lim = 0xffffffffull;
+    const long long K = (long long)a.C0 + a.C1;
+    if (a.M < 1 || a.N < 1) why = "empty";
+    else if (a.C0 < 32 || a.C0 % SG_BK) why = "C0 not a multiple of 32";
+    else if (a.C1 < 0 || a.C1 % SG_BK) why = "C1 not a multiple of 32";
+    else if (a.pix0 < a.C0 || a.pix0 % 4 || (a.C1 && (a.pix1 < a.C1 || a.pix1 % 4)) || a.out_stride < a.N) why = "bad stride";
+    else if ((unsigned long long)a.M * a.pix0 * 4ull >= lim || (unsigned long long)a.M * a.pix1 * 4ull >= lim ||
+             (unsigned long long)split3_comp_elems((size_t)a.N, (size_t)K) * 2ull >= lim || 32ull * a.out_stride * 4ull >= lim)
+        why = "beyond the 32-bit offset range";
+    if (why_not) *why_not = why;
+    return !why;
+}
+
+int gemm_split3a_blocks(long long M, int N, int cus, bool walk) {
+    const long long units = (M + 255) / 256;
+    long long per_xcd = 0;
+    for (int x = 0; x < 8; ++x) per_xcd = std::max(per_xcd, (x + 1) * units / 8 - x * units / 8);
+    long long blocks = 8 * per_xcd * ((N + 127) / 128);
+    if (walk) blocks = std::min<long long>(blocks, std::max(8, cus));
+    return blocks >= 0x7fffffffll ? -1 : (int)blocks;
+}
+
+Split3aArgs split3_1x1_args(const ConvParams& p, const unsigned short* w3) {
+    Split3aArgs a;
+    a.in0 = p.in0; a.C0 = p.C0; a.pix0 = p.pix0;
+    a.in1 = p.C1 ? p.in1 : nullptr; a.C1 = p.C1; a.pix1 = p.C1 ? p.pix1 : 0;
+    a.w3 = w3; a.bias = p.bias; a.out = p.out;
+    a.M = p.B * p.Ho * p.Wo; a.N = p.Cout; a.out_stride = p.out_stride;
+    return a;
+}
+
+static constexpr long long kSplit3x1MinRows = 2048;
+static constexpr int kSplit3x1MinK = 128, kSplit3x1MinCout = 128;
+static constexpr double kSplit3x1MinFlop = 1e10;
+Split3x1Choice split3_1x1_choose(const ConvParams& p, bool exact_f32, int master, int knob, int cus) {
+    Split3x1Choice c;
+    const long long M = (long long)p.B * p.Ho * p.Wo;
+    const char* why = nullptr;
+    if (!exact_f32) why = "not the exact-fp32 engine";
+    else if (master <= 0) why = "IRSDE_SPLIT3 = 0";
+    else if (knob <= 0) why = "IRSDE_SPLIT3_1X1 = 0";
+    else if (p.KH != 1 || p.KW != 1) why = "not a 1x1 convolution";
+    else if (p.stride != 1) why = "stride";
+    else if (p.in_shift) why = "in_shift";
+    else if (p.pad_y || p.pad_x) why = "padding";
+    else if (p.film) why = "film";
+    else if (p.silu) why = "silu";
+    else if (p.res) why = "res";
+    else if (p.in_scale) why = "in_scale";
+    else if (p.ch_scale) why = "ch_scale";
+    else if (p.gate || p.gate_film) why = "gate";
+    else if (p.shuffle) why = "shuffle";
+    else if (p.ln_g) why = "ln_g";
+    else if (p.in_bf16 || p.out_bf16 || p.in_f16 || p.out_f16) why = "16-bit storage";
+    else if (p.w_bf || p.w_pair) why = "16-bit operands";
+    else if (p.splits > 1) why = "split-K";
+    else if (p.nz != 1) why = "batched";
+    else if (M < 1 || M >= 0x7fffffffll) why = "empty";
+    else gemm_split3a_fits(split3_1x1_args(p, nullptr), &why);
+    if (!why && knob == 1) {
+        const int K = p.C0 + p.C1;
+        if (M < kSplit3x1MinRows) why = "rule: rows";
+        else if (K < kSplit3x1MinK) why = "rule: K";
+        else if (p.Cout < kSplit3x1MinCout) why = "rule: Cout";
+        else if (2.0 * (double)M * K * p.Cout < kSplit3x1MinFlop) why = "rule: FLOP";
+    }
+    if (why) {
+        c.why_not = why;
+        return c;
+    }
+    c.adopt = true;
+    c.grid = gemm_split3a_blocks(M, p.Cout, cus, true);
+    c.lds = (int)kSplit3aLds;
+    return c;
+}
+
+template <int ABL>
+static void launch_split3a_abl(bool walk, bool drain, dim3 grid, hipStream_t s, const Split3aArgs& g) {
+    if (drain) hipLaunchKernelGGL((gemm_split3a_kernel<ABL, true, true>), grid, dim3(512), kSplit3aLds, s, g);
+    else if (walk) hipLaunchKernelGGL((gemm_split3a_kernel<ABL, true>), grid, dim3(512), kSplit3aLds, s, g);
+    else hipLaunchKernelGGL((gemm_split3a_kernel<ABL, false>), grid, dim3(512), kSplit3aLds, s, g);
+}
+void launch_gemm_split3a(const Split3aArgs& a, hipStream_t s, const Split3Launch& o) {
+    const char* why = nullptr;
+    if (!gemm_split3a_fits(a, &why)) throw HipError(std::string("gemm_split3a: ") + why);
+    if (!a.in0 || (a.C1 && !a.in1) || !a.w3 || !a.out) throw HipError("gemm_split3a: null operand");
+    const bool walk = o.walk != Split3Launch::OFF, drain = o.drain == Split3Launch::ON;
+    if (drain && !walk) throw HipError("gemm_split3a: the drain twin exists on the walk only");
+    Split3aArgs g = a;
+    g.nblk_n = (a.N + 127) / 128;
+    const int forced = g_force_split3_blocks.load(std::memory_order_relaxed);
+    const int blocks = gemm_split3a_blocks(a.M, a.N, forced > 0 ? forced : device_cu_count(), walk);
+    if (blocks < 1) throw HipError("gemm_split3a: grid too large");
+    const dim3 grid((unsigned)blocks);
+    switch (o.abl) {
+        case Split3Launch::FULL: launch_split3a_abl<0>(walk, drain, grid, s, g); break;
+#ifdef IRSDE_PROBES
+        case Split3Launch::NO_LOADS: launch_split3a_abl<1>(walk, drain, grid, s, g); break;
+        case Split3Launch::NO_MFMA: launch_split3a_abl<3>(walk, drain, grid, s, g); break;
+        case Split3Launch::NO_STORES: launch_split3a_abl<4>(walk, drain, grid, s, g); break;
+#endif
+        default: throw HipError("gemm_split3a: the ablation twins are part of the PROBES build");
+    }
+    IRSDE_HIP_CHECK(hipGetLastError());
+}
+
 void launch_split_triples(const float* in, unsigned short* out, int ncomp, size_t rows, int K, hipStream_t s) {
     if (K % 32 || ncomp < 1 || rows < 1) throw HipError("split_triples: K must be a multiple of 32");
     const size_t n = (size_t)ncomp * rows * (size_t)K;
diff --git a/include/irsde_hip_debug.h b/include/irsde_hip_debug.h
--- a/include/irsde_hip_debug.h
+++ b/include/irsde_hip_debug.h
@@ -35,6 +35,11 @@
 int irsde_debug_force_split3(int mode);
 int irsde_debug_force_split3_attn(int mode);
 int irsde_debug_force_split3_blocks(int n);
+int irsde_debug_force_split3_1x1(int mode);
+int irsde_debug_split3_1x1(const float* in0, int C0, int pix0, const float* in1, int C1, int pix1, const float* w, const float* bias, float* out, int M, int N,
+                           int out_stride, int mode, void* stream);
+int irsde_debug_split3_1x1_choice(int B, int Hin, int Win, int C0, int C1, int Cout, int K, int stride, int pad, int in_shift, int operand, int storage, int pair,
+                                  unsigned features, int splits, int nz, int engine_flags, int master, int knob, int cu_count, char* out, int out_len);
 
 int irsde_debug_scam(const float* x, int B_pairs, int H, int W, int C, const float* norm_l_g, const float* norm_r_g, const float* l_proj1_w,
                      const float* l_proj1_b, const float* r_proj1_w, const float* r_proj1_b, const float* l_proj2_w, const float* l_proj2_b,
```

New measurement: 5.182 images/s, median of 6. +3.7%, better.
